# ZhengyiLuo/UHC

Measured on AMD Instinct MI355X. Metric: env-steps/sec (69-DoF SMPL humanoid, 15 substeps/step), higher is better.
Workload: dtype f64

## Files before the change

### __graft_entry__.py

```python
import os
import subprocess
import sys

ROOT = os.path.dirname(os.path.abspath(__file__))
CSRC = os.path.join(ROOT, "uhc_amd", "csrc")
LIB = os.path.join(CSRC, "libuhc_amd.so")
HIP_SOURCES = ["uhc_k_fast.hip", "uhc_k_fast_dense.hip", "uhc_k_fast_fwd.hip", "uhc_k_fast_fwd_dense.hip", "uhc_k_general.hip", "uhc_k_general_fwd.hip", "uhc_k_big.hip", "uhc_k_big_fwd.hip", "uhc_k_general_q.hip", "uhc_k_big_q.hip", "uhc_k_huge_q.hip",
               "uhc_batch_kernels.hip", "uhc_env.hip", "uhc_rollout.hip", "uhc_plan.cpp", "uhc_capi.cpp", "uhc_env_capi.cpp"]
HIP_HEADERS = ["uhc_physics_impl.h", "uhc_primal.h", "uhc_mpr.h", "uhc_device.h", "uhc_device_env.h", "uhc_host.h", "uhc_plan.h", "uhc_launch.h"]


def _stale(out, deps):
    return (not os.path.exists(out)) or any(os.path.getmtime(d) > os.path.getmtime(out) for d in deps)


def compile_lib(lib=LIB, extra_flags=(), force=False, obj_dir=None):
    from concurrent.futures import ThreadPoolExecutor
    hipcc = os.environ.get("HIPCC", "/opt/rocm/bin/hipcc")
    obj_dir = obj_dir or os.path.join(CSRC, "build")
    os.makedirs(obj_dir, exist_ok=True)
    abi = os.path.join(ROOT, "include", "uhc_amd.h")

    def deps(src):
        if src.startswith("uhc_k_"):
            big = ["uhc_primal.h"] if src.startswith(("uhc_k_big", "uhc_k_huge")) else []
            return [os.path.join(CSRC, h) for h in ["uhc_physics_impl.h", "uhc_mpr.h", "uhc_device.h", "uhc_launch.h"] + big] + [abi]
        if src == "uhc_batch_kernels.hip":
            return [os.path.join(CSRC, h) for h in ["uhc_physics_impl.h", "uhc_mpr.h", "uhc_device.h"]] + [abi]
        if src in ("uhc_env.hip", "uhc_env_capi.cpp"):
            return [os.path.join(CSRC, "uhc_device_env.h"), abi]
        if src in ("uhc_plan.cpp", "uhc_capi.cpp"):
            return [os.path.join(CSRC, h) for h in ["uhc_plan.h", "uhc_host.h", "uhc_device.h"] + (["uhc_launch.h"] if src == "uhc_capi.cpp" else [])] + [abi]
        return [abi]

    flags = ["--offload-arch=gfx950", "-O3", "-std=c++17", "-fPIC", "-fvisibility=hidden", "-Wno-unused-value"] + list(extra_flags)
    import hashlib

    def key_of(src):
        h = hashlib.sha256(" ".join(flags).encode())
        for f in [os.path.join(CSRC, src)] + deps(src):
            h.update(open(f, "rb").read())
        return h.hexdigest()

    jobs = []
    for src in HIP_SOURCES:
        sp, ob = os.path.join(CSRC, src), os.path.join(obj_dir, src + ".o")
        key = key_of(src)
        have = open(ob + ".key").read() if os.path.exists(ob + ".key") and os.path.exists(ob) else None
        if force or have != key:
            jobs.append(([hipcc] + flags + ["-c", sp, "-o", ob], ob, key))

    def run(job):
        cmd, ob, key = job
        if os.path.exists(ob + ".key"):
            os.remove(ob + ".key")
        rc = subprocess.call(cmd, cwd=CSRC)
        if rc == 0:
            open(ob + ".key", "w").write(key)
        return rc

    if jobs:
        with ThreadPoolExecutor(max_workers=min(len(jobs), os.cpu_count() or 1)) as ex:
            for rc, job in zip(ex.map(run, jobs), jobs):
                if rc != 0:
                    raise RuntimeError("hipcc failed: " + " ".join(job[0]))
    objs = [os.path.join(obj_dir, src + ".o") for src in HIP_SOURCES]
    if force or jobs or _stale(lib, objs):
        subprocess.check_call([hipcc, "--offload-arch=gfx950", "-shared", "-fPIC", "-fvisibility=hidden", "-o", lib] + objs, cwd=CSRC)


def build(force: bool = False) -> None:
    if ROOT not in sys.path:
        sys.path.insert(0, ROOT)
    compile_lib(force=force)
    from oracle.build import build as build_oracle
    build_oracle(force=force)
    import uhc_amd
    from uhc_amd import _lib
    L = _lib.lib()
    for s in _lib.SYMBOLS:
        getattr(L, s)
    lint()


def lint() -> None:
    out = os.path.join(CSRC, "build", "isa_lint.txt")
    if os.path.exists(out) and os.path.getmtime(out) >= os.path.getmtime(LIB):
        txt = open(out).read()
    else:
        r = subprocess.run([sys.executable, os.path.join(ROOT, "tools", "isa_lint.py"), LIB], capture_output=True, text=True)
# ... 52 lines not shown
```

### uhc_amd/csrc/uhc_capi.cpp

```cpp
#include <hip/hip_runtime.h>

#include <algorithm>
#include <cstdarg>
#include <cstdio>
#include <cstdlib>
#include <cstring>
#include <memory>
#include <string>
#include <vector>

#include "uhc_host.h"
#include "uhc_launch.h"
#include "uhc_plan.h"

static const UhcStepInstance g_steps[] = UHC_STEP_TABLE;
static hipError_t uhc_launch_step(int mode, int tier, const KernelArgs* A, const double* d_action, const double* d_tbase, const int* d_active,
                                  size_t lds_bytes, hipStream_t stream) {
    const bool queue = A->list != nullptr;
    if (queue) { mode = 0; tier = tier == 4 ? 4 : tier == 3 ? 3 : 2; }
    else if (tier == 3) mode = mode == 0 ? 0 : 1;
    else if (tier != 1) { tier = 2; mode = mode == 0 ? 0 : mode == 1 ? 1 : 2; }
    else mode = mode == 2 ? 2 : mode == 0 ? 0 : 1;
    const bool dense = tier != 1 || (mode != 2 && (A->cf.ndense > 0 || A->ball_limits));
    for (const UhcStepInstance& s : g_steps)
        if (s.queue == queue && s.tier == tier && s.mode == mode && s.dense == dense) return s.launch(A, d_action, d_tbase, d_active, lds_bytes, stream);
    return hipErrorInvalidDeviceFunction;
}
static hipError_t uhc_set_lds_limit(size_t lds_bytes, size_t lds_bytes_fast, size_t lds_bytes_big) {
    const size_t bytes[3] = {lds_bytes, lds_bytes_fast, lds_bytes_big};
    for (const UhcStepInstance& s : g_steps) {
        if (s.lds == 2 && !lds_bytes_big) continue;
        const hipError_t e = s.set_lds(bytes[s.lds]);
        if (e != hipSuccess) return e;
    }
    return hipSuccess;
}
extern "C" hipError_t uhc_launch_tier_lists(const int* tier, const int* d_active, int n_env, int* tier_now, int* lists, int* counts, int* cursors, int* fin,
                                            const int* cost, const int* fresh, int* order, int launch4, int* pend3, hipStream_t stream);
extern "C" hipError_t uhc_launch_gate(const int* started, int want, int* waited, long long* trace, hipStream_t stream);
extern "C" hipError_t uhc_launch_set_state(const DevState* s, int nq, int nv, int nu, const int* env_ids, int n,
                                           const double* qpos, const double* qvel, int* mask, hipStream_t stream);

static thread_local std::string g_err;
static int fail(const char* fmt, ...) {
    char buf[1024];
    va_list ap;
    va_start(ap, fmt);
    vsnprintf(buf, sizeof buf, fmt, ap);
    va_end(ap);
    g_err = buf;
    return 1;
}
#define HIP_OK(expr)                                                                      \
    do {                                                                                  \
        hipError_t e__ = (expr);                                                          \
        if (e__ != hipSuccess) return fail("%s: %s", #expr, hipGetErrorString(e__));      \
    } while (0)

extern "C" const char* uhc_last_error(void) { return g_err.c_str(); }
extern "C" int32_t uhc_abi_version(void) { return UHC_ABI_VERSION; }
extern "C" int32_t uhc_build_flags(void) {
    int32_t f = 0;
#ifdef UHC_EXPERIMENTS
    f |= 1;
#endif
#ifdef UHC_STAGE_PROF
    f |= 2;
#endif
#ifdef UHC_POISON_LDS
    f |= 4;
#endif
#ifdef UHC_GUARD_LDS
    f |= 8;
#endif
    return f;
}

template <class T>
static void take(std::vector<T>& v, const T*& p, size_t n) {
    v.assign(p, p + n);
    if (v.empty()) v.push_back(T());
    p = v.data();
}

extern "C" int32_t uhc_model_create(const UhcModelDesc* in, UhcModel** out) {
    if (!in || !out) return fail("uhc_model_create: null argument");
    if (in->nbody < 1 || in->nbody > UHC_WAVE) return fail("uhc_model_create: nbody=%d outside [1,64]", in->nbody);
    if (in->nv < 1 || in->nv > 2 * UHC_WAVE) return fail("uhc_model_create: nv=%d outside [1,128]", in->nv);
    if (in->njnt > 2 * UHC_WAVE) return fail("uhc_model_create: njnt=%d > 128", in->njnt);
    UhcModel* m = new UhcModel();
    m->d = *in;
    UhcModelDesc& d = m->d;
    const size_t nb = d.nbody, nj = d.njnt, nv = d.nv, ng = d.ngeom;
    take(m->body_parentid, d.body_parentid, nb); take(m->body_jntadr, d.body_jntadr, nb);
    take(m->body_jntnum, d.body_jntnum, nb); take(m->body_dofadr, d.body_dofadr, nb); take(m->body_dofnum, d.body_dofnum, nb);
    take(m->body_pos, d.body_pos, 3 * nb); take(m->body_quat, d.body_quat, 4 * nb); take(m->body_ipos, d.body_ipos, 3 * nb);
    take(m->body_iquat, d.body_iquat, 4 * nb); take(m->body_mass, d.body_mass, nb); take(m->body_inertia, d.body_inertia, 3 * nb);
    take(m->body_invweight0, d.body_invweight0, 2 * nb);
    take(m->jnt_type, d.jnt_type, nj); take(m->jnt_bodyid, d.jnt_bodyid, nj); take(m->jnt_qposadr, d.jnt_qposadr, nj);
    take(m->jnt_dofadr, d.jnt_dofadr, nj); take(m->jnt_limited, d.jnt_limited, nj);
    take(m->jnt_pos, d.jnt_pos, 3 * nj); take(m->jnt_axis, d.jnt_axis, 3 * nj); take(m->jnt_range, d.jnt_range, 2 * nj);
    take(m->jnt_stiffness, d.jnt_stiffness, nj); take(m->jnt_margin, d.jnt_margin, nj);
    take(m->qpos0, d.qpos0, d.nq); take(m->qpos_spring, d.qpos_spring, d.nq);
    take(m->dof_bodyid, d.dof_bodyid, nv); take(m->dof_jntid, d.dof_jntid, nv); take(m->dof_parentid, d.dof_parentid, nv);
    take(m->dof_madr, d.dof_madr, nv + 1);
    take(m->dof_armature, d.dof_armature, nv); take(m->dof_damping, d.dof_damping, nv);
    take(m->dof_frictionloss, d.dof_frictionloss, nv); take(m->dof_invweight0, d.dof_invweight0, nv);
    take(m->geom_type, d.geom_type, ng); take(m->geom_bodyid, d.geom_bodyid, ng); take(m->geom_contype, d.geom_contype, ng);
    take(m->geom_conaffinity, d.geom_conaffinity, ng); take(m->geom_condim, d.geom_condim, ng);
    take(m->geom_vertadr, d.geom_vertadr, ng); take(m->geom_vertnum, d.geom_vertnum, ng);
    take(m->geom_pos, d.geom_pos, 3 * ng); take(m->geom_quat, d.geom_quat, 4 * ng); take(m->geom_size, d.geom_size, 3 * ng);
    take(m->geom_friction, d.geom_friction, 3 * ng); take(m->geom_margin, d.geom_margin, ng); take(m->geom_gap, d.geom_gap, ng);
    take(m->geom_solref, d.geom_solref, 2 * ng); take(m->geom_solimp, d.geom_solimp, 5 * ng);
    take(m->geom_rbound, d.geom_rbound, ng); take(m->geom_center, d.geom_center, 3 * ng);
    take(m->mesh_vert, d.mesh_vert, 3 * (size_t)d.nmeshvert);
    take(m->mesh_adjadr, d.mesh_adjadr, (size_t)d.nmeshvert + 1); take(m->mesh_adj, d.mesh_adj, d.nmeshadj);
    take(m->exclude_pair, d.exclude_pair, 2 * (size_t)d.nexclude);
    take(m->actuator_dofid, d.actuator_dofid, d.nu); take(m->actuator_gear, d.actuator_gear, 3 * (size_t)d.nu);
    for (size_t b = 1; b < nb; b++)
        if (d.body_parentid[b] >= (int)b) { delete m; return fail("uhc_model_create: bodies must be in depth-first order"); }
    for (size_t i = 0; i < nv; i++)
        if (d.dof_parentid[i] >= (int)i) { delete m; return fail("uhc_model_create: dofs must be in depth-first order"); }
    *out = m;
    return 0;
}
extern "C" void uhc_model_free(UhcModel* m) { delete m; }
extern "C" int32_t uhc_model_nM(const UhcModel* m) { return m ? m->d.dof_madr[m->d.nv] : -1; }

template <class T>
static int upload(UhcBatch* b, const std::vector<T>& h, const T** dptr) {
    void* p = nullptr;
    size_t bytes = std::max<size_t>(h.size(), 1) * sizeof(T);
    HIP_OK(hipMalloc(&p, bytes));
    b->allocs.push_back(p);
    if (!h.empty()) HIP_OK(hipMemcpy(p, h.data(), h.size() * sizeof(T), hipMemcpyHostToDevice));
    *dptr = (const T*)p;
    return 0;
}
template <class T>
static int dalloc(UhcBatch* b, size_t n, T** dptr) {
    void* p = nullptr;
    const size_t bytes = std::max<size_t>(n, 1) * sizeof(T);
    if (b->hbm_guard) {
        HIP_OK(hipMalloc(&p, bytes + 512));
        HIP_OK(hipMemset(p, 0xA5, bytes + 512));
        HIP_OK(hipMemset((char*)p + 256, 0, bytes));
        b->allocs.push_back(p);
        b->fences.push_back({(char*)p, bytes});
        *dptr = (T*)((char*)p + 256);
        return 0;
    }
    HIP_OK(hipMalloc(&p, bytes));
    HIP_OK(hipMemset(p, 0, bytes));
    b->allocs.push_back(p);
    *dptr = (T*)p;
    return 0;
}
#define TRY(x) do { if (x) return 1; } while (0)


static int upload_plan(UhcBatch* b, const BatchPlan& P, const UhcModelDesc& d, const UhcCtrlDesc* ctrl, const int32_t* h_env_model) {
    KernelArgs& A = b->A;
    DevTopo& T = A.t;
    const int nb = d.nbody, nv = d.nv, nj = d.njnt, ng = d.ngeom;
    auto ivec = [](const int32_t* p, size_t n) { return std::vector<int>(p, p + n); };
    TRY(upload(b, ivec(d.body_parentid, nb), &T.body_parentid)); TRY(upload(b, ivec(d.body_jntadr, nb), &T.body_jntadr));
    TRY(upload(b, ivec(d.body_jntnum, nb), &T.body_jntnum)); TRY(upload(b, ivec(d.body_dofadr, nb), &T.body_dofadr));
    TRY(upload(b, ivec(d.body_dofnum, nb), &T.body_dofnum)); TRY(upload(b, P.body_rootid, &T.body_rootid));
    TRY(upload(b, P.body_nsub, &T.body_nsub)); TRY(upload(b, P.body_lastdof, &T.body_lastdof)); TRY(upload(b, P.body_depth, &T.body_depth));
    TRY(upload(b, ivec(d.jnt_type, nj), &T.jnt_type)); TRY(upload(b, ivec(d.jnt_bodyid, nj), &T.jnt_bodyid));
    TRY(upload(b, ivec(d.jnt_qposadr, nj), &T.jnt_qposadr)); TRY(upload(b, ivec(d.jnt_dofadr, nj), &T.jnt_dofadr));
    TRY(upload(b, ivec(d.jnt_limited, nj), &T.jnt_limited));
    TRY(upload(b, ivec(d.dof_bodyid, nv), &T.dof_bodyid)); TRY(upload(b, ivec(d.dof_jntid, nv), &T.dof_jntid));
    TRY(upload(b, ivec(d.dof_parentid, nv), &T.dof_parentid)); TRY(upload(b, ivec(d.dof_madr, nv + 1), &T.dof_madr));
    TRY(upload(b, P.dof_depth, &T.dof_depth)); TRY(upload(b, P.dof_ndesc, &T.dof_ndesc));
    TRY(upload(b, P.dof_anc, &T.dof_anc)); TRY(upload(b, P.ncommon, &T.dof_ncommon)); TRY(upload(b, P.m_row, &T.m_row)); TRY(upload(b, P.m_col, &T.m_col)); TRY(upload(b, P.m_ij, &T.m_ij));
    TRY(upload(b, ivec(d.geom_type, ng), &T.geom_type)); TRY(upload(b, ivec(d.geom_bodyid, ng), &T.geom_bodyid));
    TRY(upload(b, ivec(d.geom_condim, ng), &T.geom_condim)); TRY(upload(b, ivec(d.geom_vertadr, ng), &T.geom_vertadr));
    TRY(upload(b, ivec(d.geom_vertnum, ng), &T.geom_vertnum));
    TRY(upload(b, P.pg1, &T.pair_g1)); TRY(upload(b, P.pg2, &T.pair_g2));
    TRY(upload(b, P.cg1, &T.cpair_g1)); TRY(upload(b, P.cg2, &T.cpair_g2)); TRY(upload(b, P.dof_rootid, &T.dof_rootid));
    TRY(upload(b, ivec(d.actuator_dofid, d.nu), &T.actuator_dofid));
    TRY(upload(b, P.model_blob, &A.s.model_blob));
    if (h_env_model) TRY(upload(b, std::vector<int>(h_env_model, h_env_model + b->n_env), &A.s.env_model));
    else if (b->n_models > 1) TRY(upload(b, std::vector<int>(b->n_env, 0), &A.s.env_model));
    if (A.c.rfc_mode == 2) TRY(upload(b, P.vf_body, &A.c.vf_body));
    auto dvec = [&](const double* p) { return std::vector<double>(p, p + d.nu); };
    TRY(upload(b, dvec(ctrl->jkp), &A.c.jkp)); TRY(upload(b, dvec(ctrl->jkd), &A.c.jkd));
    TRY(upload(b, dvec(ctrl->torque_lim), &A.c.torque_lim)); TRY(upload(b, dvec(ctrl->a_scale), &A.c.a_scale));
    if (!P.guard_tab.empty()) {
        const std::vector<int>& tab = P.guard_tab;
        int* d_tab = nullptr;
        TRY(dalloc(b, tab.size(), &d_tab)); TRY(dalloc(b, 4, &b->d_guard_hits));
        HIP_OK(hipMemcpy(d_tab, tab.data(), tab.size() * sizeof(int), hipMemcpyHostToDevice));
        HIP_OK(hipMemset(b->d_guard_hits, 0, 4 * sizeof(int)));
        A.guard_tab = d_tab; A.guard_hits = b->d_guard_hits;
        fprintf(stderr, "uhc guard: LDS guard words on -- fast %d + %d, general %d + %d, large %d + %d, tier 4 %d + %d (persistent + constraint phase)\n", tab[0], tab[1],
                tab[64], tab[65], tab[128], tab[129], tab[192], tab[193]);
    }
    TRY(upload(b, P.chain, &T.chain));
    TRY(upload(b, P.dof_act, &T.dof_act));
    TRY(upload(b, P.fac_prog, &T.fac_prog)); TRY(upload(b, P.sol_back, &T.sol_back)); TRY(upload(b, P.sol_fwd, &T.sol_fwd));
    return 0;
}

static int alloc_state(UhcBatch* b, const UhcModel* const* models, const int32_t* h_env_model) {
    KernelArgs& A = b->A;
    DevState& S = A.s;
    const size_t E = b->n_env;
    const int nq = A.t.nq, nv = A.t.nv, nu = A.t.nu, nb = A.t.nbody;
    TRY(dalloc(b, E * nq, &S.qpos)); TRY(dalloc(b, E * nv, &S.qvel)); TRY(dalloc(b, E * nv, &S.qacc)); TRY(dalloc(b, E * nv, &S.qacc_ws));
    TRY(dalloc(b, E * 3 * nb, &S.xpos)); TRY(dalloc(b, E * 4 * nb, &S.xquat)); TRY(dalloc(b, E * 3 * nb, &S.xipos));
    TRY(dalloc(b, 4, &S.path_stats));
    TRY(dalloc(b, E * A.t.nM, &S.qM)); TRY(dalloc(b, 6 * E + 1, &S.redo)); S.pend2 = S.redo + E; S.pend3 = S.redo + 2 * E; S.resume = S.redo + 3 * E; S.why = S.redo + 4 * E; TRY(dalloc(b, 2, &S.q_abort));
    A.chunk_done = S.redo + 5 * E; A.ticket = S.redo + 6 * E; TRY(dalloc(b, E * UHC_CHUNK_REC, &A.chunk_rec));
    TRY(dalloc(b, E, &S.tier)); TRY(dalloc(b, E, &b->tier_now)); S.tier_now = b->tier_now; TRY(dalloc(b, E, &S.cost));
    if (!(A.dbg & 8)) TRY(dalloc(b, E, &b->d_order));
    TRY(dalloc(b, 3 * E, &b->d_lists)); TRY(dalloc(b, 8, &b->d_counts)); TRY(dalloc(b, 8, &b->d_cursors)); TRY(dalloc(b, 8, &b->d_fin));
    { std::vector<int> one(E, 1); HIP_OK(hipMemcpy(S.tier, one.data(), E * sizeof(int), hipMemcpyHostToDevice)); } TRY(dalloc(b, E, &S.fresh)); TRY(dalloc(b, E * 40, &S.prof)); TRY(dalloc(b, E * nv, &S.bias)); TRY(dalloc(b, E * nu, &S.ctrl));
    TRY(dalloc(b, E * nv, &S.applied));
    if (A.c.rfc_mode == 2) { TRY(dalloc(b, E * 6 * nv, &S.cdof)); TRY(dalloc(b, E * 3 * nb, &S.rootcom)); }
    TRY(dalloc(b, E, &S.ncon)); TRY(dalloc(b, E, &S.nefc)); TRY(dalloc(b, E, &S.fail)); TRY(dalloc(b, E, &S.solver_iter));
    TRY(dalloc(b, E, &S.overflow));
    if (A.last_tier == 4) { TRY(dalloc(b, E * (size_t)A.gy_stride, &A.gY)); TRY(dalloc(b, E * (size_t)A.gd_stride, &A.gD)); }
    TRY(dalloc(b, E, &b->reset_mask));
    {
        std::vector<double> q0(E * nq);
        for (size_t e = 0; e < E; e++) {
            const UhcModelDesc& md = models[h_env_model ? h_env_model[e] : 0]->d;
            memcpy(&q0[e * nq], md.qpos0, nq * sizeof(double));
        }
        HIP_OK(hipMemcpy(S.qpos, q0.data(), q0.size() * sizeof(double), hipMemcpyHostToDevice));
    }
    const int64_t n = (int64_t)E;
    const UhcBatch::Field fields[21] = {{S.qpos, n * nq}, {S.qvel, n * nv}, {S.xpos, n * 3 * nb}, {S.xquat, n * 4 * nb}, {S.xipos, n * 3 * nb}, {S.qM, n * A.t.nM}, {S.bias, n * nv},
                                        {S.qacc, n * nv}, {S.ctrl, n * nu}, {S.ncon, n}, {S.nefc, n}, {S.fail, n}, {S.solver_iter, n}, {S.applied, n * nv}, {S.overflow, n},
                                        {S.prof, n * 40}, {S.redo, n}, {S.tier, n}, {S.why, n}, {S.qacc_ws, n * nv}, {S.cost, n}};
    std::copy(fields, fields + 21, b->field);
    return 0;
}

extern "C" void uhc_batch_free(UhcBatch* b);
extern "C" int32_t uhc_batch_create(const UhcModel* const* models, int32_t n_models, const int32_t* h_env_model, int32_t n_env,
                                    int32_t device_id, const UhcCtrlDesc* ctrl, UhcBatch** out) {
    if (!out) return fail("uhc_batch_create: bad argument");
    const BatchKnobs knobs = read_knobs();
    BatchPlan P;
    std::string err;
    if (plan_batch(models, n_models, h_env_model, n_env, ctrl, knobs, &P, &err)) return fail("%s", err.c_str());
    int ndev = 0;
    HIP_OK(hipGetDeviceCount(&ndev));
    if (device_id < 0 || device_id >= ndev) return fail("uhc_batch_create: device %d not present (%d devices)", device_id, ndev);
    HIP_OK(hipSetDevice(device_id));

    std::unique_ptr<UhcBatch, void (*)(UhcBatch*)> owner(new UhcBatch(), uhc_batch_free);
    UhcBatch* b = owner.get();
    b->n_env = n_env;
    b->device = device_id;
    b->n_models = n_models;
    b->n_trailing_free = P.n_trailing_free;
    b->A = P.A;
    b->nM = P.A.t.nM;
    b->lds_bytes = P.lds_bytes; b->lds_bytes_fast = P.lds_bytes_fast; b->lds_bytes_big = P.lds_bytes_big;
    b->use_fast = P.use_fast;
    b->hbm_guard = knobs.guard != 0;
    b->q2_div = knobs.q2_div; b->q2_wait_min = knobs.q2_wait_min; b->q2_max = knobs.q2_max; b->q3_max = knobs.q3_max; b->q4_max = knobs.q4_max;
    b->fast_chunk = (P.A.dbg & 4) ? 0x7fff : knobs.fast_chunk;
    TRY(upload_plan(b, P, models[0]->d, ctrl, h_env_model));
    HIP_OK(uhc_set_lds_limit(b->lds_bytes, b->lds_bytes_fast, b->lds_bytes_big));
    TRY(alloc_state(b, models, h_env_model));
    HIP_OK(hipStreamCreateWithFlags(&b->own_stream, hipStreamNonBlocking));
    b->stream = b->own_stream;
    *out = owner.release();
    return 0;
}

static void guard_report(UhcBatch* b) {
    if (!b->d_guard_hits) return;
    int h[4] = {0, 0, 0, 0};
    if (hipMemcpy(h, b->d_guard_hits, sizeof(h), hipMemcpyDeviceToHost) != hipSuccess) return;
    if (h[0] > b->guard_reported) {
        b->guard_reported = h[0];
        fprintf(stderr, "uhc guard: %d LDS guard words OVERWRITTEN so far; the first: tier %d, %s region %d (offset %d doubles), env %d\n", h[0], h[1] >> 16,
                ((h[1] >> 8) & 0xff) ? "constraint-phase" : "persistent", h[1] & 0xff, h[3], h[2]);
    }
}
extern "C" void uhc_batch_free(UhcBatch* b) {
    if (!b) return;
    hipSetDevice(b->device);
    hipDeviceSynchronize();
    guard_report(b);
    if (!b->fences.empty()) {
        int bad = 0;
        unsigned char h[512];
        for (size_t k = 0; k < b->fences.size(); k++) {
            const auto& f = b->fences[k];
            bool hit = false;
            if (hipMemcpy(h, f.first, 256, hipMemcpyDeviceToHost) != hipSuccess || hipMemcpy(h + 256, f.first + 256 + f.second, 256, hipMemcpyDeviceToHost) != hipSuccess) continue;
            for (int i = 0; i < 512; i++) hit = hit || h[i] != 0xA5;
            if (hit) { if (!bad) fprintf(stderr, "uhc guard: HBM array %zu (%zu bytes) has an OVERWRITTEN fence\n", k, f.second); bad++; }
        }
        fprintf(stderr, "uhc guard: %zu fenced HBM arrays checked, %d with an overwritten fence\n", b->fences.size(), bad);
    }
    if (b->d_guard_hits) fprintf(stderr, "uhc guard: batch of %d envs freed, %d guard words overwritten in its lifetime\n", b->n_env, b->guard_reported);
    for (void* p : b->allocs) hipFree(p);
    for (auto& ev : b->ev_used) { hipEventDestroy(ev.first); hipEventDestroy(ev.second); }
    for (auto& ev : b->ev_free) { hipEventDestroy(ev.first); hipEventDestroy(ev.second); }
    for (hipEvent_t e : {b->ev_fork, b->ev_side1, b->ev_side2, b->ev_side3}) if (e) hipEventDestroy(e);
    for (hipEvent_t e : b->cnt_ev) if (e) hipEventDestroy(e);
    if (b->h_counts) hipHostFree(b->h_counts);
    if (b->side_stream) hipStreamDestroy(b->side_stream);
    if (b->side_stream3) hipStreamDestroy(b->side_stream3);
    if (b->side_stream4) hipStreamDestroy(b->side_stream4);
    if (b->own_stream) hipStreamDestroy(b->own_stream);
    delete b;
}
extern "C" int32_t uhc_batch_set_stream(UhcBatch* b, void* s) {
    if (!b) return fail("uhc_batch_set_stream: null batch");
    b->stream = (hipStream_t)s;
    return 0;
}
extern "C" int32_t uhc_batch_sync(UhcBatch* b) {
    if (!b) return fail("uhc_batch_sync: null batch");
    HIP_OK(hipStreamSynchronize(b->stream));
    guard_report(b);
    return 0;
}
extern "C" int32_t uhc_batch_set_rfc_scale(UhcBatch* b, double s) {
    if (!b) return fail("uhc_batch_set_rfc_scale: null batch");
    b->A.c.rfc_scale = s;
    return 0;
}
extern "C" int32_t uhc_batch_set_kernel_path(UhcBatch* b, int32_t mode) {
    if (!b) return fail("uhc_batch_set_kernel_path: null batch");
    if (mode < 0 || mode > 2) return fail("uhc_batch_set_kernel_path: mode %d (0 fast then general, 1 general only, 2 adaptive)", mode);
    b->general_only = mode == 1;
    b->path_mode = mode;
    if (mode == 2 && !b->side_stream) {
        HIP_OK(hipSetDevice(b->device));
        int least = 0, greatest = 0;
        HIP_OK(hipDeviceGetStreamPriorityRange(&least, &greatest));
        HIP_OK(hipStreamCreateWithPriority(&b->side_stream, hipStreamNonBlocking, greatest));
        HIP_OK(hipStreamCreateWithPriority(&b->side_stream3, hipStreamNonBlocking, (least != greatest && least != 0) ? least : greatest));
        b->large_first = least != greatest && least != 0;
        { hipDeviceProp_t pr; HIP_OK(hipGetDeviceProperties(&pr, b->device)); b->n_cu = pr.multiProcessorCount > 0 ? pr.multiProcessorCount : 256; }
        HIP_OK(hipHostMalloc((void**)&b->h_counts, sizeof(int) * 8 * 8, hipHostMallocDefault));
        memset(b->h_counts, 0, sizeof(int) * 8 * 8);
        for (int k = 0; k < 8; k++) HIP_OK(hipEventCreateWithFlags(&b->cnt_ev[k], hipEventDisableTiming));
        HIP_OK(hipEventCreateWithFlags(&b->ev_fork, hipEventDisableTiming));
        HIP_OK(hipEventCreateWithFlags(&b->ev_side1, hipEventDisableTiming));
        HIP_OK(hipEventCreateWithFlags(&b->ev_side2, hipEventDisableTiming));
        HIP_OK(hipStreamCreateWithPriority(&b->side_stream4, hipStreamNonBlocking, (least != greatest && least != 0) ? least : greatest));
        HIP_OK(hipEventCreateWithFlags(&b->ev_side3, hipEventDisableTiming));
    }
    return 0;
}
extern "C" int32_t uhc_batch_set_solver(UhcBatch* b, int32_t solver, int32_t iterations) {
    if (!b || (solver != 0 && solver != 1)) return fail("uhc_batch_set_solver: solver must be 0 (sweeps) or 1 (active set)");
    b->A.t.solver = solver;
    if (iterations > 0) b->A.t.iterations = iterations;
    return 0;
}
extern "C" int32_t uhc_batch_field(UhcBatch* b, int32_t f, void** p, int64_t* n) {
    if (!b || f < 0 || f > 20 || !b->field[f].ptr) return fail("uhc_batch_field: unknown field %d", f);
    if (p) *p = b->field[f].ptr;
    if (n) *n = b->field[f].count;
    return 0;
}
static int launch_sticky(UhcBatch* b, int mode, const double* d_action, const double* d_tbase, const int* d_active, bool timed, std::pair<hipEvent_t, hipEvent_t> ev) {
    const bool big = b->A.last_tier >= 3;
        KernelArgs K = b->A;
        int est4 = 0, est2_then = 0;
        if (b->A.last_tier == 4 && b->q4_max > 0)
            for (long long k = b->cnt_step - 1; k >= 0 && k > b->cnt_step - 8; k--)
                if (hipEventQuery(b->cnt_ev[k % 8]) == hipSuccess) { est4 = b->h_counts[8 * (k % 8) + 7]; est2_then = b->h_counts[8 * (k % 8) + 2]; break; }
        (void)hipGetLastError();
    StickyInputs in{};
    in.est4 = est4; in.est2_then = est2_then; in.n_env = b->n_env; in.n_cu = b->n_cu; in.lds_bytes_fast = b->lds_bytes_fast; in.large_first = b->large_first;
    in.fast_chunk = b->fast_chunk; in.n_substeps = b->A.c.n_substeps;
    in.last_tier = b->A.last_tier; in.q2_div = b->q2_div; in.q2_wait_min = b->q2_wait_min; in.q2_max = b->q2_max; in.q3_max = b->q3_max; in.q4_max = b->q4_max;
#ifdef UHC_EXPERIMENTS
    in.fixed_cap2 = (b->A.dbg & 2048) != 0;
#endif
    in.queues_off = b->queues_off;
    const bool launch4 = plan_sticky_step(in).launch4;
        K.cnt4 = b->d_counts + 7;
        HIP_OK(uhc_launch_tier_lists(b->A.s.tier, d_active, b->n_env, b->tier_now, b->d_lists, b->d_counts, b->d_cursors, b->d_fin, b->A.s.cost, b->A.s.fresh, b->d_order,
                                     launch4 ? 1 : 0, b->A.s.pend3, b->stream));
        HIP_OK(hipEventRecord(b->ev_fork, b->stream));
        if (b->cnt_step >= 2) HIP_OK(hipEventSynchronize(b->cnt_ev[(b->cnt_step - 2) % 8]));
        int est2 = 0, est3 = 0, handed2 = 0;
        for (long long k = b->cnt_step - 1; k >= 0 && k > b->cnt_step - 8; k--)
            if (hipEventQuery(b->cnt_ev[k % 8]) == hipSuccess) {
                const int* hc = b->h_counts + 8 * (k % 8);
                est2 = hc[2]; est3 = hc[3]; handed2 = std::max(0, hc[2] - hc[4]);
                if (b->A.dbg & 64) fprintf(stderr, "uhc step %lld: queues %d / %d envs (%d handed on), gate waited %.1f us, gave up %d, queues_off %d\n", k, est2, est3, handed2, 0.01 * hc[1], hc[0], (int)b->queues_off);
                if (hc[0] > b->aborts_seen) {
                    b->aborts_seen = hc[0];
                    b->queues_off_until = ++b->abort_events >= 3 ? (long long)1 << 62 : b->cnt_step + 32;
                }
                b->queues_off = b->cnt_step < b->queues_off_until;
                break;
            }
    in.est2 = est2; in.est3 = est3; in.handed2 = handed2; in.queues_off = b->queues_off;
    const StickySizes z = plan_sticky_step(in);
    const bool queues = z.queues, waiting = z.waiting, q3 = z.q3, q4 = launch4 && q3;
    const int grid2 = z.grid2, grid3 = z.grid3, grid4 = z.grid4;
    K.sticky_mask = (queues ? 4 : 0) | (q3 ? 8 : 0) | (launch4 ? 16 : 0);
        if (q4) {
            HIP_OK(hipStreamWaitEvent(b->side_stream4, b->ev_fork, 0));
            K.tier_want = 0; K.list = b->d_lists + 2 * b->n_env; K.list_count = b->d_counts + 6; K.list_cursor = b->d_cursors + 4;
            K.grid = grid4; K.n_wait = grid4; K.spares = nullptr; K.started = nullptr;
            K.prod_fin = b->d_fin + 5; K.prod_total = grid3;
            K.fin = nullptr; K.q_next = nullptr; K.q_next_count = nullptr;
            if (b->A.dbg & 64) fprintf(stderr, "uhc step %lld: %d tier-4 consumers (%d env-steps went through tier 4 when last seen)\n", b->cnt_step, grid4, est4);
            HIP_OK(uhc_launch_step(mode, 4, &K, d_action, d_tbase, nullptr, b->lds_bytes_big, b->side_stream4));
            HIP_OK(hipEventRecord(b->ev_side3, b->side_stream4));
        }
        auto launch_large = [&]() -> int {
            HIP_OK(hipStreamWaitEvent(b->side_stream3, b->ev_fork, 0));
            K.tier_want = 0; K.list = b->d_lists + b->n_env; K.list_count = b->d_counts + 3; K.list_cursor = b->d_cursors + 3;
            K.grid = grid3; K.n_wait = grid3; K.spares = nullptr; K.started = b->d_fin + 4;
            K.prod_fin = b->d_fin + 2; K.prod_total = grid2;
            K.fin = q4 ? b->d_fin + 5 : nullptr; K.q_next = q4 ? b->d_lists + 2 * b->n_env : nullptr; K.q_next_count = q4 ? b->d_counts + 6 : nullptr;
            HIP_OK(uhc_launch_step(mode, 3, &K, d_action, d_tbase, nullptr, b->lds_bytes_big, b->side_stream3));
            HIP_OK(hipEventRecord(b->ev_side2, b->side_stream3));
            return 0;
        };
        if (q3 && b->large_first) { if (launch_large()) return -1; }
        if (queues) {
            HIP_OK(hipStreamWaitEvent(b->side_stream, b->ev_fork, 0));
            if (q3 && b->large_first && !(b->A.dbg & 32)) HIP_OK(uhc_launch_gate(b->d_fin + 4, grid3, nullptr, nullptr, b->side_stream));
            K.tier_want = 0; K.list = b->d_lists; K.list_count = b->d_counts + 2; K.list_cursor = b->d_cursors + 2;
            K.grid = grid2;
            K.prod_fin = waiting ? b->d_fin + 1 : nullptr; K.prod_total = z.fast.prod_total;
            K.fin = b->d_fin + 2; K.started = waiting ? b->d_fin + 3 : nullptr;
            K.n_wait = z.n_wait; K.spares = b->d_fin;
            K.q_next = q3 ? b->d_lists + b->n_env : nullptr; K.q_next_count = q3 ? b->d_counts + 3 : nullptr;
            HIP_OK(uhc_launch_step(mode, 2, &K, d_action, d_tbase, nullptr, b->lds_bytes, b->side_stream));
            HIP_OK(hipEventRecord(b->ev_side1, b->side_stream));
        }
        if (q3 && !b->large_first) { if (launch_large()) return -1; }
        K.list = nullptr; K.list_count = nullptr; K.list_cursor = nullptr; K.grid = 0; K.prod_fin = nullptr; K.prod_total = 0; K.started = nullptr; K.spares = nullptr;
        if (waiting && !(b->A.dbg & 32)) HIP_OK(uhc_launch_gate(b->d_fin + 3, grid2, b->d_counts + 1,
                                                                     (b->A.dbg & 16) ? b->A.s.prof + (size_t)(b->n_env - 1) * 40 + 16 : nullptr, b->stream));
        K.tier_want = 1;
        K.chunk = z.fast.chunk; K.grid = z.fast.chunk ? z.fast.grid : 0;
        K.order = b->d_order;
        K.fin = waiting ? b->d_fin + 1 : nullptr;
        K.q_next = waiting ? b->d_lists : nullptr; K.q_next_count = waiting ? b->d_counts + 2 : nullptr;
        if (timed) HIP_OK(hipEventRecord(ev.first, b->stream));
        HIP_OK(uhc_launch_step(mode, 1, &K, d_action, d_tbase, d_active, b->lds_bytes_fast, b->stream));
        if (timed) { HIP_OK(hipEventRecord(ev.second, b->stream)); b->ev_used.push_back(ev); }
        K.tier_want = 0; K.sticky_mask = 0; K.fin = nullptr; K.q_next = nullptr; K.q_next_count = nullptr; K.order = nullptr; K.chunk = 0; K.grid = 0;
        if (queues) HIP_OK(hipStreamWaitEvent(b->stream, b->ev_side1, 0));
        HIP_OK(uhc_launch_step(mode, 2, &K, d_action, d_tbase, b->A.s.pend2, b->lds_bytes, b->stream));
        if (q3) HIP_OK(hipStreamWaitEvent(b->stream, b->ev_side2, 0));
        if (q4) HIP_OK(hipStreamWaitEvent(b->stream, b->ev_side3, 0));
        if (big) HIP_OK(uhc_launch_step(mode, 3, &K, d_action, d_tbase, b->A.s.pend3, b->lds_bytes_big, b->stream));
        const int slot = (int)(b->cnt_step % 8);
        HIP_OK(hipMemcpyAsync(b->d_counts, b->A.s.q_abort, sizeof(int), hipMemcpyDeviceToDevice, b->stream));
        HIP_OK(hipMemcpyAsync(b->h_counts + 8 * slot, b->d_counts, 8 * sizeof(int), hipMemcpyDeviceToHost, b->stream));
        HIP_OK(hipEventRecord(b->cnt_ev[slot], b->stream));
        b->cnt_step++;
        return 0;
    }

static int launch(UhcBatch* b, int mode, const double* d_action, const double* d_tbase, const int* d_active) {
    std::pair<hipEvent_t, hipEvent_t> ev{nullptr, nullptr};
    const bool timed = b->timing && mode == 0;
    if (timed) {
        if (b->ev_free.empty()) { HIP_OK(hipEventCreate(&ev.first)); HIP_OK(hipEventCreate(&ev.second)); }
        else { ev = b->ev_free.back(); b->ev_free.pop_back(); }
    }
    const bool general = b->general_only;
    const bool big = b->A.last_tier >= 3;
    HIP_OK(hipMemsetAsync(b->A.s.redo, 0, sizeof(int) * ((size_t)b->n_env * 6 + 1), b->stream));
    bool capturing = false;
    {
        hipStreamCaptureStatus cs = hipStreamCaptureStatusNone;
        if (hipStreamIsCapturing(b->stream, &cs) == hipSuccess) capturing = cs == hipStreamCaptureStatusActive;
        else (void)hipGetLastError();
    }
    if (mode == 0 && b->path_mode == 2 && b->use_fast && !general && !capturing) return launch_sticky(b, mode, d_action, d_tbase, d_active, timed, ev);
    if (b->use_fast && !general) {
        if (timed) HIP_OK(hipEventRecord(ev.first, b->stream));
        KernelArgs K = b->A;
        if (mode == 0) {
            const FastChunks f = plan_fast_chunks(K.c.n_substeps, default_fast_chunk(b->fast_chunk, K.c.n_substeps, b->n_env, b->n_cu, b->lds_bytes_fast), b->n_env);
            K.chunk = f.chunk; K.grid = f.chunk ? f.grid : 0;
        }
        HIP_OK(uhc_launch_step(mode, 1, &K, d_action, d_tbase, d_active, b->lds_bytes_fast, b->stream));
        if (timed) { HIP_OK(hipEventRecord(ev.second, b->stream)); b->ev_used.push_back(ev); }
        HIP_OK(uhc_launch_step(mode, 2, &b->A, d_action, d_tbase, b->A.s.pend2, b->lds_bytes, b->stream));
    } else {
        if (timed) HIP_OK(hipEventRecord(ev.first, b->stream));
        HIP_OK(uhc_launch_step(mode, 2, &b->A, d_action, d_tbase, d_active, b->lds_bytes, b->stream));
        if (timed) { HIP_OK(hipEventRecord(ev.second, b->stream)); b->ev_used.push_back(ev); }
    }
    if (big) HIP_OK(uhc_launch_step(mode, 3, &b->A, d_action, d_tbase, b->A.s.pend3, b->lds_bytes_big, b->stream));
    return 0;
}

extern "C" int32_t uhc_batch_set_overflow_mode(UhcBatch* b, int32_t truncate) {
    if (!b) return fail("uhc_batch_set_overflow_mode: null batch");
    b->A.truncate = truncate != 0;
    return 0;
}
extern "C" int32_t uhc_batch_set_timing(UhcBatch* b, int32_t enable) {
    if (!b) return fail("uhc_batch_set_timing: null batch");
    b->timing = enable != 0;
    return 0;
}
extern "C" int32_t uhc_batch_kernel_time(UhcBatch* b, double* total_ms, int32_t* launches) {
    if (!b || !total_ms || !launches) return fail("uhc_batch_kernel_time: null argument");
    double tot = 0;
    for (auto& ev : b->ev_used) {
        float ms = 0;
        HIP_OK(hipEventSynchronize(ev.second));
        HIP_OK(hipEventElapsedTime(&ms, ev.first, ev.second));
        tot += ms;
        b->ev_free.push_back(ev);
// ... 62 lines not shown
```

### uhc_amd/csrc/uhc_device.h

```cpp
#pragma once
#include <hip/hip_runtime.h>
#include <stdint.h>

#define UHC_WAVE 64
#define UHC_FAST_MAXEFC 64
#define UHC_FAST_MAXCON 16
#define UHC_FAST_MAXCON_DENSE 24
#define UHC_FAST_MAXTWO 12
#define UHC_GEN_MAXEFC 128
#define UHC_GEN_MAXCON 64
#define UHC_GEN_MAXTWO 20
#define UHC_BIG_MAXEFC 256
#define UHC_BIG_MAXCON 128
#define UHC_BIG_MAXTWO 32
#define UHC_MAXTWO 32
#define UHC_HUGE_MAXEFC 1024
#define UHC_HUGE_MAXCON 192
#define UHC_HUGE_MAXCON_MOST 320
#define UHC_HUGE_MAXTWO 128
#define UHC_DOF_MAXACT 4
#define UHC_CON_STRIDE 24
#define UHC_WHY_CONTACTS (1 << 16)
#define UHC_WHY_ROWS (1 << 17)
#define UHC_WHY_DENSE_SLOTS (1 << 18)
// ... 76 lines not shown
    int* q_abort;
    int* tier;
    const int* tier_now;
    int* cost;
    int* fresh;
    const int* env_model;
    long long* prof;
    unsigned long long* path_stats;
    const double* model_blob;
};

#define UHC_PRIMAL_WAVES 4
#define UHC_PRIMAL_CLS_STRIDE 144
struct PrimalScratch { int anc, stY, dstage, pair_all, pair_cls, pair_cnt, cw, mbx, part, runs, total; };
__host__ __device__ inline PrimalScratch primal_scratch(int nv, int YS) {
    PrimalScratch p;
    int o = 0;
    auto take = [&](int n) { const int at = o; o += (n + 1) & ~1; return at; };
    p.anc = take((nv * YS + 3) / 4 + 1);
    p.stY = take(UHC_PRIMAL_WAVES * 16 * 32);
    p.dstage = take(nv * 8);
    p.pair_all = take(528 / 4);
    p.pair_cls = take(4 * UHC_PRIMAL_CLS_STRIDE / 4);
    p.pair_cnt = take((4 * 33 + 3) / 4);
    p.cw = take(UHC_PRIMAL_WAVES * 32);
    p.mbx = take(4);
    p.part = take(UHC_PRIMAL_WAVES * 128);
    p.runs = take(UHC_HUGE_MAXEFC / 2);
    p.total = o;
    return p;
}

struct TierCap {
    int maxefc, maxcon;
    int ndense;
    int ycap;
    int vstage;
    int ld_delta;
};
struct KernelArgs {
    DevTopo t;
    DevNumOff o;
    DevLds lf;
    DevLds l;
    DevLds lh;
    DevLds lx;
    TierCap cf, cg, ch, cx;
    double* gY;
    double* gD;
    int gy_stride, gd_stride;
    int last_tier;
    const int* order;
    int tier_want;
    int sticky_mask;
    int* list;
    int* list_count;
    int* list_cursor;
    const int* prod_fin;
    int prod_total;
    int n_wait;
    int* spares;
    int* started;
    int* fin;
    int* q_next;
    int* q_next_count;
    const int* guard_tab;
    int* guard_hits;
    int* cnt4;
    int grid;
    int marks[8];
    int t4_rows;
    int truncate;
    int ball_limits;
    int dbg;
    int nvp;
    int adjdeg;
    DevCtrl c;
    DevState s;
    int n_env;
    int chunk;
    int* ticket;
    int* chunk_done;
    int* chunk_rec;
};
#define UHC_CHUNK_ALL 0x7fff
#define UHC_CHUNK_ABANDON (1 << 30)
#define UHC_CHUNK_TAKEN (1 << 29)
#define UHC_CHUNK_CLOSING (1 << 28)
#define UHC_CHUNK_REC 16
```

### uhc_amd/csrc/uhc_host.h

```cpp
#pragma once
#include <hip/hip_runtime.h>

#include <cstdint>
#include <utility>
#include <vector>

#include "../../include/uhc_amd.h"
#include "uhc_device.h"

struct UhcModel {
    UhcModelDesc d;
    std::vector<int32_t> body_parentid, body_jntadr, body_jntnum, body_dofadr, body_dofnum;
    std::vector<double> body_pos, body_quat, body_ipos, body_iquat, body_mass, body_inertia, body_invweight0;
    std::vector<int32_t> jnt_type, jnt_bodyid, jnt_qposadr, jnt_dofadr, jnt_limited;
    std::vector<double> jnt_pos, jnt_axis, jnt_range, jnt_stiffness, jnt_margin, qpos0, qpos_spring;
    std::vector<int32_t> dof_bodyid, dof_jntid, dof_parentid, dof_madr;
    std::vector<double> dof_armature, dof_damping, dof_frictionloss, dof_invweight0;
    std::vector<int32_t> geom_type, geom_bodyid, geom_contype, geom_conaffinity, geom_condim, geom_vertadr, geom_vertnum;
    std::vector<double> geom_pos, geom_quat, geom_size, geom_friction, geom_margin, geom_gap, geom_solref, geom_solimp,
        geom_rbound, geom_center, mesh_vert;
    std::vector<int32_t> mesh_adjadr, mesh_adj, exclude_pair, actuator_dofid;
    std::vector<double> actuator_gear;
};

struct UhcBatch {
    int n_env = 0, device = 0;
    hipStream_t own_stream = nullptr, stream = nullptr;
    KernelArgs A;
    size_t lds_bytes = 0, lds_bytes_fast = 0, lds_bytes_big = 0;
    bool use_fast = true;
    bool general_only = false;
    int path_mode = 0;
    hipStream_t side_stream = nullptr, side_stream3 = nullptr, side_stream4 = nullptr;
    hipEvent_t ev_fork = nullptr, ev_side1 = nullptr, ev_side2 = nullptr, ev_side3 = nullptr;
    int* tier_now = nullptr;
    bool large_first = false;
    int n_cu = 256;
    std::vector<std::pair<char*, size_t>> fences;
    int* d_guard_hits = nullptr;
    int guard_reported = 0;
    int* d_order = nullptr;
    int aborts_seen = 0, abort_events = 0;
    long long queues_off_until = 0;
    int q2_wait_min = 16;
    int q2_div = 1;
    int q2_max = 256;
    int q4_max = 16;
    int q3_max = 32;
    int fast_chunk = 0;
    int *d_lists = nullptr, *d_counts = nullptr, *d_cursors = nullptr, *d_fin = nullptr;
    bool queues_off = false;
    int* h_counts = nullptr;
    hipEvent_t cnt_ev[8] = {};
    long long cnt_step = 0;
    std::vector<void*> allocs;
    int nM = 0;
    int* reset_mask = nullptr;
    bool timing = false;
    std::vector<std::pair<hipEvent_t, hipEvent_t>> ev_used, ev_free;
    int n_models = 1;
    int n_trailing_free = 0;
    bool hbm_guard = false;
    struct Field { void* ptr; int64_t count; };
    Field field[21] = {};
};
```

### uhc_amd/csrc/uhc_launch.h

```cpp
#pragma once
#include <hip/hip_runtime.h>

#include "uhc_device.h"

typedef hipError_t (*UhcStepLaunch)(const KernelArgs* A, const double* d_action, const double* d_tbase, const int* d_active, size_t lds_bytes, hipStream_t stream);
typedef hipError_t (*UhcSetLds)(size_t lds_bytes);

#define UHC_STEP_INSTANCES(X)                                                                                                                     \
    X(m0_fast, 0, 1, false, false) X(m0_fast_dense, 0, 1, true, false) X(m1_fast, 1, 1, false, false) X(m1_fast_dense, 1, 1, true, false)         \
    X(m2_fast, 2, 1, false, false) X(m0_gen, 0, 2, true, false) X(m1_gen, 1, 2, true, false) X(m2_gen, 2, 2, true, false)                         \
    X(m0_big, 0, 3, true, false) X(m1_big, 1, 3, true, false) X(m0_gen_q, 0, 2, true, true) X(m0_big_q, 0, 3, true, true) X(m0_huge_q, 0, 4, true, true)

#define UHC_DECL_LAUNCH(name, mode, tier, dense, queue)                                                                                         \
    extern "C" hipError_t uhc_launch_##name(const KernelArgs* A, const double* d_action, const double* d_tbase, const int* d_active, size_t lds_bytes, \
                                            hipStream_t stream);                                                                                 \
    extern "C" hipError_t uhc_launch_##name##_lds(size_t lds_bytes);
UHC_STEP_INSTANCES(UHC_DECL_LAUNCH)

#define UHC_DEFINE_LAUNCH(name, KERNEL, MODE, TIER, DENSE, THREADS, GRID, ...)                                                                        \
    extern "C" hipError_t uhc_launch_##name(const KernelArgs* A, const double* d_action, const double* d_tbase, const int* d_active, size_t lds_bytes, \
                                            hipStream_t stream) {                                                                                     \
        (void)d_active;                                                                                                                               \
        hipLaunchKernelGGL((KERNEL<MODE, TIER, DENSE>), dim3(GRID), dim3(THREADS), lds_bytes, stream, *A, d_action, d_tbase, ##__VA_ARGS__);          \
        return hipGetLastError();                                                                                                                     \
    }                                                                                                                                                 \
    extern "C" hipError_t uhc_launch_##name##_lds(size_t lds_bytes) {                                                                                 \
        return hipFuncSetAttribute((const void*)KERNEL<MODE, TIER, DENSE>, hipFuncAttributeMaxDynamicSharedMemorySize, (int)lds_bytes);               \
    }
#define UHC_ENV_LAUNCH(name, MODE, TIER, DENSE) UHC_DEFINE_LAUNCH(name, uhc_step_kernel, MODE, TIER, DENSE, UHC_WAVE, A->grid ? A->grid : A->n_env, d_active)
#define UHC_QUEUE_LAUNCH(name, TIER, THREADS) UHC_DEFINE_LAUNCH(name, uhc_step_queue_kernel, 0, TIER, true, THREADS, A->grid)

struct UhcStepInstance { int mode, tier; bool dense, queue; UhcStepLaunch launch; UhcSetLds set_lds; int lds; };
#define UHC_INSTANCE_ROW(name, mode, tier, dense, queue) {mode, tier, dense, queue, uhc_launch_##name, uhc_launch_##name##_lds, tier == 1 ? 1 : tier == 2 ? 0 : 2},
#define UHC_STEP_TABLE {UHC_STEP_INSTANCES(UHC_INSTANCE_ROW)}
```

### uhc_amd/csrc/uhc_mpr.h

```cpp
#pragma once

#define UHC_CCD_EPS 2.220446049250313e-16
#define UHC_MPR_TOLERANCE 1e-6
#define UHC_MPR_MAXIT 50
#define UHC_MPR_MAXSUP 256

struct V3 { double x, y, z; };
__device__ __forceinline__ V3 v3(double x, double y, double z) { V3 r = {x, y, z}; return r; }
__device__ __forceinline__ V3 operator-(const V3& a, const V3& b) { return v3(a.x - b.x, a.y - b.y, a.z - b.z); }
__device__ __forceinline__ V3 operator+(const V3& a, const V3& b) { return v3(a.x + b.x, a.y + b.y, a.z + b.z); }
__device__ __forceinline__ V3 operator*(const V3& a, double s) { return v3(a.x * s, a.y * s, a.z * s); }
__device__ __forceinline__ V3 neg(const V3& a) { return v3(-a.x, -a.y, -a.z); }
__device__ __forceinline__ double vdot(const V3& a, const V3& b) { return a.x * b.x + a.y * b.y + a.z * b.z; }
__device__ __forceinline__ V3 vcross(const V3& a, const V3& b) { return v3(a.y * b.z - a.z * b.y, a.z * b.x - a.x * b.z, a.x * b.y - a.y * b.x); }
__device__ __forceinline__ V3 vnorm(const V3& a) { const double n = sqrt(vdot(a, a)); return v3(a.x / n, a.y / n, a.z / n); }
__device__ __forceinline__ V3 vsel(bool c, const V3& a, const V3& b) { return v3(c ? a.x : b.x, c ? a.y : b.y, c ? a.z : b.z); }
__device__ __forceinline__ bool ccd_zero(double x) { return fabs(x) < UHC_CCD_EPS; }
__device__ __forceinline__ bool ccd_eq(double a, double b) {
    const double ab = fabs(a - b);
    if (ab < UHC_CCD_EPS) return true;
    a = fabs(a); b = fabs(b);
    return b > a ? ab < UHC_CCD_EPS * b : ab < UHC_CCD_EPS * a;
}

// ... 312 lines not shown
                    pair_support_wave2(VB, Ap, Aq, a, b, a2, b2v);
                    const bool mq = LANE == q;
                    v4.v = vsel(mq, a2 - b2v, v4.v);
                    v4.s = vsel(mq, a2 + b2v, v4.s);
                    const bool mine = LANE == p;
                    v4.v = vsel(mine, a - b, v4.v);
                    v4.s = vsel(mine, a + b, v4.s);
                    continue;
                }
            }
            pair_support_wave(VB, Ap.R1, Ap.P1, Ap.voff1, Ap.vn1, Ap.R2, Ap.P2, Ap.voff2, Ap.vn2, Ap.d, Ap.hm1, Ap.hm2, a, b);
            const bool mine = LANE == p;
            v4.v = vsel(mine, a - b, v4.v);
            v4.s = vsel(mine, a + b, v4.s);
        }
        bool to_refine = false, to_pen = false;
        if (st == MPR_D1) {
            p1 = v4;
            dt = vdot(p1.v, dir);
            if (ccd_zero(dt) || dt < 0) st = MPR_DONE;
            else {
                dir = vcross(p0.v, p1.v);
                if (ccd_zero(vdot(dir, dir))) {
                    if (ccd_eq(p1.v.x, 0) && ccd_eq(p1.v.y, 0) && ccd_eq(p1.v.z, 0)) { M.depth = 0; M.dir = v3(0, 0, 0); }
                    else { M.depth = sqrt(vdot(p1.v, p1.v)); M.dir = vnorm(p1.v); }
                    M.pos = v3(0.5 * p1.s.x, 0.5 * p1.s.y, 0.5 * p1.s.z);
                    M.hit = true;
                    st = MPR_DONE;
                } else { dir = vnorm(dir); st = MPR_D2; }
            }
        } else if (st == MPR_D2) {
            p2 = v4;
            dt = vdot(p2.v, dir);
            if (ccd_zero(dt) || dt < 0) st = MPR_DONE;
            else {
                dir = vnorm(vcross(p1.v - p0.v, p2.v - p0.v));
                if (vdot(dir, p0.v) > 0) { const CcdSup t = p1; p1 = p2; p2 = t; dir = neg(dir); }
                st = MPR_D3;
            }
        } else if (st == MPR_D3) {
            dt = vdot(v4.v, dir);
            if (ccd_zero(dt) || dt < 0) st = MPR_DONE;
            else {
                bool cont = false;
                dt = vdot(vcross(p1.v, v4.v), p0.v);
                if (dt < 0 && !ccd_zero(dt)) { p2 = v4; cont = true; }
                if (!cont) {
                    dt = vdot(vcross(v4.v, p2.v), p0.v);
                    if (dt < 0 && !ccd_zero(dt)) { p1 = v4; cont = true; }
                }
                if (cont) dir = vnorm(vcross(p1.v - p0.v, p2.v - p0.v));
                else { p3 = v4; to_refine = true; }
            }
        } else if (st == MPR_REFINE) {
            dt = vdot(v4.v, dir);
            if (!(ccd_zero(dt) || dt > 0) || portal_reach_tolerance(p1, p2, p3, v4, dir)) st = MPR_DONE;
            else { expand_portal(p0, p1, p2, p3, v4); to_refine = true; }
        } else if (st == MPR_PEN) {
            if (portal_reach_tolerance(p1, p2, p3, v4, dir) || it > UHC_MPR_MAXIT) {
                V3 pd;
                M.depth = sqrt(point_tri_dist2(p1.v, p2.v, p3.v, pd));
                if (ccd_zero(pd.x) && ccd_zero(pd.y) && ccd_zero(pd.z)) pd = dir;
                M.dir = vnorm(pd);
                M.pos = find_pos(p0, p1, p2, p3);
                M.hit = true;
                st = MPR_DONE;
            } else {
                expand_portal(p0, p1, p2, p3, v4);
                it++;
                dir = portal_dir(p1, p2, p3);
            }
        }
        if (to_refine) {
            dir = portal_dir(p1, p2, p3);
            dt = vdot(dir, p1.v);
            if (ccd_zero(dt) || dt > 0) to_pen = true;
            else st = MPR_REFINE;
        }
        if (to_pen) { dir = portal_dir(p1, p2, p3); it = 0; st = MPR_PEN; }
    }
}

#if defined(UHC_NW2)
enum { MCMD_EXIT = 0, MCMD_ROUND = 1, MCMD_ROWS = 2 };
struct MprMB { int* hdr; double* io[6]; double* hm1; double* hm2; int* st4; int* st2; };
template <int TIER>
__device__ __forceinline__ MprMB mpr_mb(const KernelArgs& A, double* S) {
    const DevLds& L = lds_of<TIER>(A);
    MprMB m;
    m.hdr = (int*)(S + L.rowR);
    m.io[0] = S + L.rowR + 4;
    m.io[1] = S + L.rowAref; m.io[2] = S + L.rowAref + UHC_WAVE;
    m.io[3] = S + L.rowB; m.io[4] = S + L.rowB + UHC_WAVE;
    m.io[5] = S + L.rowF; m.hm1 = S + L.rowF + UHC_WAVE;
    m.st4 = (int*)(S + L.rowDa); m.st2 = (int*)(S + L.rowW); m.hm2 = S + L.rowW + UHC_WAVE;
    return m;
}
__device__ __forceinline__ SupArgs mpr_mb_args(const MprMB& MB, const double* xmat, const double* xpos, int p) {
    SupArgs a;
    const int b1 = __builtin_amdgcn_readfirstlane(MB.st4[4 * p]), b2 = __builtin_amdgcn_readfirstlane(MB.st4[4 * p + 1]);
    a.R1 = xmat + 9 * b1; a.P1 = xpos + 3 * b1; a.R2 = xmat + 9 * b2; a.P2 = xpos + 3 * b2;
    a.voff1 = __builtin_amdgcn_readfirstlane(MB.st4[4 * p + 2]); a.vn1 = __builtin_amdgcn_readfirstlane(MB.st4[4 * p + 3]);
    a.voff2 = __builtin_amdgcn_readfirstlane(MB.st2[2 * p]); a.vn2 = __builtin_amdgcn_readfirstlane(MB.st2[2 * p + 1]);
    a.hm1 = MB.hm1[p]; a.hm2 = MB.hm2[p];
    a.d = v3(MB.io[0][p], MB.io[1][p], MB.io[2][p]);
    return a;
}
__device__ __forceinline__ void mpr_mb_put(const MprMB& MB, int p, const V3& a, const V3& b) {
    if (LANE == 0) {
        MB.io[0][p] = a.x - b.x; MB.io[1][p] = a.y - b.y; MB.io[2][p] = a.z - b.z; MB.io[3][p] = a.x + b.x; MB.io[4][p] = a.y + b.y; MB.io[5][p] = a.z + b.z;
    }
}
__device__ __forceinline__ void mpr_serve_round(const double* __restrict__ VB, const double* __restrict__ xmat, const double* __restrict__ xpos, const MprMB& MB, unsigned long long live, int wid, int nw) {
    const int n = __builtin_popcountll(live), h = (n + nw - 1) / nw;
    int take = min(h, n - wid * h);
    for (int k = 0; k < wid * h && live; k++) live &= live - 1;
    while (live && take > 0) {
        const int p = __ffsll((long long)live) - 1;
        live &= live - 1;
        const SupArgs Ap = mpr_mb_args(MB, xmat, xpos, p);
        V3 a, b;
        if (take >= 2 && live && UHC_MPR_PAIRWISE) {
            const int q = __ffsll((long long)live) - 1;
            const SupArgs Aq = mpr_mb_args(MB, xmat, xpos, q);
            if (max(max(Ap.vn1, Ap.vn2), max(Aq.vn1, Aq.vn2)) <= UHC_WAVE) {
                live &= live - 1;
                take -= 2;
                V3 a2, b2v;
                pair_support_wave2(VB, Ap, Aq, a, b, a2, b2v);
                mpr_mb_put(MB, p, a, b);
                mpr_mb_put(MB, q, a2, b2v);
                continue;
            }
        }
        pair_support_wave(VB, Ap.R1, Ap.P1, Ap.voff1, Ap.vn1, Ap.R2, Ap.P2, Ap.voff2, Ap.vn2, Ap.d, Ap.hm1, Ap.hm2, a, b);
        mpr_mb_put(MB, p, a, b);
        take -= 1;
    }
}
template <bool LDSV>
__device__ __forceinline__ void mpr_wave_mw(const double* __restrict__ VB, const double* __restrict__ xmat, const double* __restrict__ xpos, bool active, MprLane& M, const MprMB& MB, int vstage,
                                            const double* vb_global) {
    CcdSup p0, p1, p2, p3, v4;
    V3 dir = v3(0, 0, 0);
    double dt;
    int st = MPR_DONE, it = 0;
    M.hit = false; M.depth = 0; M.dir = v3(0, 0, 0); M.pos = v3(0, 0, 0);
    p0.v = p0.s = p1.v = p1.s = p2.v = p2.s = p3.v = p3.s = v4.v = v4.s = v3(0, 0, 0);
    if (active) {
        p0.s = M.c1 + M.c2; p0.v = M.c1 - M.c2;
        if (ccd_eq(p0.v.x, 0) && ccd_eq(p0.v.y, 0) && ccd_eq(p0.v.z, 0)) p0.v.x += UHC_CCD_EPS * 10;
        dir = vnorm(neg(p0.v));
        st = MPR_D1;
        MB.st4[4 * LANE] = M.b1; MB.st4[4 * LANE + 1] = M.b2; MB.st4[4 * LANE + 2] = M.voff1; MB.st4[4 * LANE + 3] = M.vn1;
        MB.st2[2 * LANE] = M.voff2; MB.st2[2 * LANE + 1] = M.vn2;
        MB.hm1[LANE] = M.hm1; MB.hm2[LANE] = M.hm2;
    }
    int* mbi = MB.hdr;
    if (LANE == 0) {
        mbi[3] = LDSV ? vstage : -1;
        mbi[4] = (int)((unsigned long long)vb_global & 0xffffffffull); mbi[5] = (int)((unsigned long long)vb_global >> 32);
    }
    for (int round = 0;; round++) {
        const unsigned long long live = __builtin_amdgcn_ballot_w64(st != MPR_DONE);
        if (!live || round == UHC_MPR_MAXSUP) break;
        if (st != MPR_DONE) { MB.io[0][LANE] = dir.x; MB.io[1][LANE] = dir.y; MB.io[2][LANE] = dir.z; }
        if (LANE == 0) { mbi[0] = MCMD_ROUND; mbi[1] = (int)(live & 0xffffffffull); mbi[2] = (int)(live >> 32); }
        __syncthreads();
        mpr_serve_round(VB, xmat, xpos, MB, live, 0, UHC_NWG);
        __syncthreads();
        if (st != MPR_DONE) { v4.v = v3(MB.io[0][LANE], MB.io[1][LANE], MB.io[2][LANE]); v4.s = v3(MB.io[3][LANE], MB.io[4][LANE], MB.io[5][LANE]); }
        bool to_refine = false, to_pen = false;
        if (st == MPR_D1) {
            p1 = v4;
            dt = vdot(p1.v, dir);
            if (ccd_zero(dt) || dt < 0) st = MPR_DONE;
            else {
                dir = vcross(p0.v, p1.v);
                if (ccd_zero(vdot(dir, dir))) {
                    if (ccd_eq(p1.v.x, 0) && ccd_eq(p1.v.y, 0) && ccd_eq(p1.v.z, 0)) { M.depth = 0; M.dir = v3(0, 0, 0); }
                    else { M.depth = sqrt(vdot(p1.v, p1.v)); M.dir = vnorm(p1.v); }
                    M.pos = v3(0.5 * p1.s.x, 0.5 * p1.s.y, 0.5 * p1.s.z);
                    M.hit = true;
                    st = MPR_DONE;
                } else { dir = vnorm(dir); st = MPR_D2; }
            }
        } else if (st == MPR_D2) {
            p2 = v4;
            dt = vdot(p2.v, dir);
            if (ccd_zero(dt) || dt < 0) st = MPR_DONE;
            else {
                dir = vnorm(vcross(p1.v - p0.v, p2.v - p0.v));
                if (vdot(dir, p0.v) > 0) { const CcdSup t = p1; p1 = p2; p2 = t; dir = neg(dir); }
                st = MPR_D3;
            }
        } else if (st == MPR_D3) {
            dt = vdot(v4.v, dir);
            if (ccd_zero(dt) || dt < 0) st = MPR_DONE;
            else {
                bool cont = false;
                dt = vdot(vcross(p1.v, v4.v), p0.v);
                if (dt < 0 && !ccd_zero(dt)) { p2 = v4; cont = true; }
                if (!cont) {
                    dt = vdot(vcross(v4.v, p2.v), p0.v);
                    if (dt < 0 && !ccd_zero(dt)) { p1 = v4; cont = true; }
                }
                if (cont) dir = vnorm(vcross(p1.v - p0.v, p2.v - p0.v));
                else { p3 = v4; to_refine = true; }
            }
        } else if (st == MPR_REFINE) {
            dt = vdot(v4.v, dir);
            if (!(ccd_zero(dt) || dt > 0) || portal_reach_tolerance(p1, p2, p3, v4, dir)) st = MPR_DONE;
            else { expand_portal(p0, p1, p2, p3, v4); to_refine = true; }
        } else if (st == MPR_PEN) {
            if (portal_reach_tolerance(p1, p2, p3, v4, dir) || it > UHC_MPR_MAXIT) {
                V3 pd;
                M.depth = sqrt(point_tri_dist2(p1.v, p2.v, p3.v, pd));
                if (ccd_zero(pd.x) && ccd_zero(pd.y) && ccd_zero(pd.z)) pd = dir;
                M.dir = vnorm(pd);
                M.pos = find_pos(p0, p1, p2, p3);
                M.hit = true;
                st = MPR_DONE;
            } else {
                expand_portal(p0, p1, p2, p3, v4);
                it++;
                dir = portal_dir(p1, p2, p3);
            }
        }
        if (to_refine) {
            dir = portal_dir(p1, p2, p3);
            dt = vdot(dir, p1.v);
            if (ccd_zero(dt) || dt > 0) to_pen = true;
            else st = MPR_REFINE;
        }
        if (to_pen) { dir = portal_dir(p1, p2, p3); it = 0; st = MPR_PEN; }
    }
}
template <int TIER>
__device__ __forceinline__ void mpr_helper(const KernelArgs& A, double* S) {
    const DevLds& L = lds_of<TIER>(A);
    const MprMB MB = mpr_mb<TIER>(A, S);
    const int* mbi = MB.hdr;
    const int wid = __builtin_amdgcn_readfirstlane((int)(threadIdx.x >> 6));
    const LaneConst HLC = lane_const<true>(A.t);
    for (;;) {
        __syncthreads();
        const int cmd = __builtin_amdgcn_readfirstlane(mbi[0]);
        if (cmd == MCMD_EXIT) return;
        if (cmd == MCMD_ROWS) {
            const int nefc = __builtin_amdgcn_readfirstlane(mbi[1]), ntwo = __builtin_amdgcn_readfirstlane(mbi[2]);
            const unsigned long long mbp = ((unsigned long long)(unsigned)__builtin_amdgcn_readfirstlane(mbi[5]) << 32) | (unsigned)__builtin_amdgcn_readfirstlane(mbi[4]);
            __syncthreads();
            if (ntwo > 0) k_dense_groups<TIER>(A, S, HLC, S + L.dense, ntwo, 1, 2);
            __syncthreads();
            if (UHC_WAVE + LANE < nefc) k_row_one<TIER>(A, (const double*)mbp, S, UHC_WAVE + LANE, S + L.Y);
            __syncthreads();
            continue;
        }
        const unsigned long long live = ((unsigned long long)(unsigned)__builtin_amdgcn_readfirstlane(mbi[2]) << 32) | (unsigned)__builtin_amdgcn_readfirstlane(mbi[1]);
        const int vst = __builtin_amdgcn_readfirstlane(mbi[3]);
        if (vst >= 0) mpr_serve_round(S + vst, S + L.xmat, S + L.xpos, MB, live, wid, UHC_NWG);
        else {
            const unsigned long long vb = ((unsigned long long)(unsigned)__builtin_amdgcn_readfirstlane(mbi[5]) << 32) | (unsigned)__builtin_amdgcn_readfirstlane(mbi[4]);
            mpr_serve_round((const double*)vb, S + L.xmat, S + L.xpos, MB, live, wid, UHC_NWG);
        }
        __syncthreads();
    }
}
template <int TIER>
__device__ __forceinline__ void mpr_release_helpers(const KernelArgs& A, double* S) {
    int* mbi = mpr_mb<TIER>(A, S).hdr;
    if (LANE == 0) mbi[0] = MCMD_EXIT;
    __syncthreads();
}
#endif
```

### uhc_amd/csrc/uhc_physics_impl.h

```cpp
#pragma once
#include <type_traits>
#include "../../include/uhc_amd.h"
#include "uhc_device.h"

extern __shared__ __attribute__((aligned(16))) double smem[];

#if defined(UHC_NW4)
#define UHC_NWG 4
#elif defined(UHC_NW2)
#define UHC_NWG 2
#else
#define UHC_NWG 1
#endif
#if UHC_NWG > 1
#define LANE ((int)(threadIdx.x & 63u))
#else
#define LANE ((int)threadIdx.x)
#endif
#define UHC_NPROF 40
#ifdef UHC_STAGE_PROF
#define PROF_DECL long long pt_[UHC_NPROF] = {}; long long pt_last_ = __builtin_readcyclecounter();
#define PROF_ARGS , long long* pt_, long long& pt_last_
#define PROF_PASS , pt_, pt_last_
#define PROF(i) { const long long now_ = __builtin_readcyclecounter(); pt_[i] += now_ - pt_last_; pt_last_ = now_; }
#else
#define PROF_DECL
#define PROF_ARGS
#define PROF_PASS
#define PROF(i)
#endif
#ifdef UHC_EXPERIMENTS
#define UHC_EXP(bit) ((A.dbg & (bit)) != 0)
#else
#define UHC_EXP(bit) false
#endif
template <int TIER> __device__ __forceinline__ const DevLds& lds_of(const KernelArgs& A) {
    if constexpr (TIER == 1) return A.lf; else if constexpr (TIER == 2) return A.l; else if constexpr (TIER == 3) return A.lh; else return A.lx;
}
template <int TIER> __device__ __forceinline__ const TierCap& cap_of(const KernelArgs& A) {
    if constexpr (TIER == 1) return A.cf; else if constexpr (TIER == 2) return A.cg; else if constexpr (TIER == 3) return A.ch; else return A.cx;
}
template <int TIER> __device__ __forceinline__ bool hands_on(const KernelArgs& A) { return TIER == 1 ? !A.truncate : TIER < A.last_tier; }
#if UHC_NWG > 1
__device__ __forceinline__ void wsync() {
    __builtin_amdgcn_fence(__ATOMIC_RELEASE, "workgroup");
    __builtin_amdgcn_wave_barrier();
    __builtin_amdgcn_fence(__ATOMIC_ACQUIRE, "workgroup");
}
#else
__device__ __forceinline__ void wsync() { __syncthreads(); }
#endif
template <int TIER> __device__ __forceinline__ double* y_store(const KernelArgs& A, double* S, int env) {
    if constexpr (TIER == 4) return A.gY + (size_t)env * A.gy_stride; else return S + lds_of<TIER>(A).Y;
}
template <int TIER> __device__ __forceinline__ double* d_store(const KernelArgs& A, double* S, int env) {
    if constexpr (TIER == 4) return A.gD + (size_t)env * A.gd_stride; else return S + lds_of<TIER>(A).dense;
}

__device__ __forceinline__ double bcast(double v, int src) {
    int lo = __builtin_amdgcn_readlane(__double2loint(v), src);
    int hi = __builtin_amdgcn_readlane(__double2hiint(v), src);
    return __hiloint2double(hi, lo);
}
template <int CTRL>
__device__ __forceinline__ double dpp_f64(double v) {
    const int lo = __builtin_amdgcn_update_dpp(0, __double2loint(v), CTRL, 0xf, 0xf, true);
    const int hi = __builtin_amdgcn_update_dpp(0, __double2hiint(v), CTRL, 0xf, 0xf, true);
    return __hiloint2double(hi, lo);
}
#define DPP_QUAD_1032 0xB1
#define DPP_QUAD_2301 0x4E
#define DPP_ROW_HALF_MIRROR 0x141
#define DPP_ROW_MIRROR 0x140
__device__ __forceinline__ double wave_sum(double v) {
    v += dpp_f64<DPP_QUAD_1032>(v);
    v += dpp_f64<DPP_QUAD_2301>(v);
    v += dpp_f64<DPP_ROW_HALF_MIRROR>(v);
    v += dpp_f64<DPP_ROW_MIRROR>(v);
    return (bcast(v, 0) + bcast(v, 16)) + (bcast(v, 32) + bcast(v, 48));
}
__device__ __forceinline__ double wave_min(double v) {
    v = fmin(v, dpp_f64<DPP_QUAD_1032>(v));
    v = fmin(v, dpp_f64<DPP_QUAD_2301>(v));
    v = fmin(v, dpp_f64<DPP_ROW_HALF_MIRROR>(v));
    v = fmin(v, dpp_f64<DPP_ROW_MIRROR>(v));
    return fmin(fmin(bcast(v, 0), bcast(v, 16)), fmin(bcast(v, 32), bcast(v, 48)));
}
__device__ __forceinline__ int wave_or(int v) { return __builtin_amdgcn_ballot_w64(v != 0) != 0; }
template <int TIER> __device__ __forceinline__ void k_row_one(const KernelArgs& A, const double* mb, double* S, const int r, double* Yb);
struct LaneConst { int d0, d1, n0, n1, m0, m1, pk0, pk1, r0, r1; bool v0, v1; };
template <int TIER> __device__ __forceinline__ void k_dense_groups(const KernelArgs& A, double* S, const LaneConst& LC, double* Db, const int ntwo, const int first, const int stride);
template <bool DENSE> __device__ __forceinline__ LaneConst lane_const(const DevTopo& T);
#include "uhc_mpr.h"

__device__ __forceinline__ void cross3(double* r, const double* a, const double* b) {
    double r0 = a[1] * b[2] - a[2] * b[1], r1 = a[2] * b[0] - a[0] * b[2], r2 = a[0] * b[1] - a[1] * b[0];
    r[0] = r0; r[1] = r1; r[2] = r2;
}
__device__ __forceinline__ double dot3(const double* a, const double* b) { return a[0] * b[0] + a[1] * b[1] + a[2] * b[2]; }
__device__ __forceinline__ void quat_mul(double* r, const double* a, const double* b) {
    double t0 = a[0] * b[0] - a[1] * b[1] - a[2] * b[2] - a[3] * b[3];
    double t1 = a[0] * b[1] + a[1] * b[0] + a[2] * b[3] - a[3] * b[2];
    double t2 = a[0] * b[2] - a[1] * b[3] + a[2] * b[0] + a[3] * b[1];
    double t3 = a[0] * b[3] + a[1] * b[2] - a[2] * b[1] + a[3] * b[0];
    r[0] = t0; r[1] = t1; r[2] = t2; r[3] = t3;
}
__device__ __forceinline__ void quat_normalize(double* q) {
    double n = sqrt(q[0] * q[0] + q[1] * q[1] + q[2] * q[2] + q[3] * q[3]);
    if (n < UHC_MINVAL) { q[0] = 1; q[1] = q[2] = q[3] = 0; return; }
    double inv = 1.0 / n;
    q[0] *= inv; q[1] *= inv; q[2] *= inv; q[3] *= inv;
}
__device__ __forceinline__ void quat_to_mat(double* m, const double* q) {
    double w = q[0], x = q[1], y = q[2], z = q[3];
    m[0] = w * w + x * x - y * y - z * z; m[1] = 2 * (x * y - w * z); m[2] = 2 * (x * z + w * y);
    m[3] = 2 * (x * y + w * z); m[4] = w * w - x * x + y * y - z * z; m[5] = 2 * (y * z - w * x);
    m[6] = 2 * (x * z - w * y); m[7] = 2 * (y * z + w * x); m[8] = w * w - x * x - y * y + z * z;
}
__device__ __forceinline__ void mat_vec(double* r, const double* m, const double* v) {
    double t0 = m[0] * v[0] + m[1] * v[1] + m[2] * v[2];
    double t1 = m[3] * v[0] + m[4] * v[1] + m[5] * v[2];
    double t2 = m[6] * v[0] + m[7] * v[1] + m[8] * v[2];
    r[0] = t0; r[1] = t1; r[2] = t2;
}
__device__ __forceinline__ void axis_angle_quat(double* q, const double* axis, double angle) {
    double s, c;
    sincos(0.5 * angle, &s, &c);
    q[0] = c; q[1] = axis[0] * s; q[2] = axis[1] * s; q[3] = axis[2] * s;
}
__device__ __forceinline__ void cross_motion(double* r, const double* v, const double* m) {
    double a[3], b[3];
    cross3(r, v, m);
    cross3(a, v, m + 3);
    cross3(b, v + 3, m);
    r[3] = a[0] + b[0]; r[4] = a[1] + b[1]; r[5] = a[2] + b[2];
}
__device__ __forceinline__ void cross_force(double* r, const double* v, const double* f) {
    double a[3], b[3];
    cross3(a, v, f);
    cross3(b, v + 3, f + 3);
    r[0] = a[0] + b[0]; r[1] = a[1] + b[1]; r[2] = a[2] + b[2];
    cross3(r + 3, v, f + 3);
}
__device__ __forceinline__ void inert_mul(double* r, const double* I, const double* v) {
    const double *w = v, *l = v + 3, *h = I + 6;
    double hxl[3], wxh[3];
    cross3(hxl, h, l);
    cross3(wxh, w, h);
    r[0] = I[0] * w[0] + I[3] * w[1] + I[4] * w[2] + hxl[0];
    r[1] = I[3] * w[0] + I[1] * w[1] + I[5] * w[2] + hxl[1];
    r[2] = I[4] * w[0] + I[5] * w[1] + I[2] * w[2] + hxl[2];
    r[3] = I[9] * l[0] + wxh[0];
    r[4] = I[9] * l[1] + wxh[1];
    r[5] = I[9] * l[2] + wxh[2];
}
__device__ __forceinline__ double dot6(const double* a, const double* b) {
    return a[0] * b[0] + a[1] * b[1] + a[2] * b[2] + a[3] * b[3] + a[4] * b[4] + a[5] * b[5];
}
__device__ __forceinline__ double clampd(double x, double lo, double hi) { return fmin(fmax(x, lo), hi); }
__device__ __forceinline__ double max0(double x) {
    double r;
    asm("v_max_f64 %0, %1, 0" : "=v"(r) : "v"(x));
    return r;
}

template <int I, int N, class F>
__device__ __forceinline__ void static_for(F&& f) {
    if constexpr (I < N) {
        f(std::integral_constant<int, I>{});
        static_for<I + 1, N>(f);
    }
}

__device__ __forceinline__ void agpr_put(int& a, int v) { asm volatile("v_accvgpr_write_b32 %0, %1" : "=a"(a) : "v"(v)); }
__device__ __forceinline__ int agpr_get(int a) { int v; asm volatile("v_accvgpr_read_b32 %0, %1" : "=v"(v) : "a"(a)); return v; }
// ... 459 lines not shown
        const int item = LANE + UHC_WAVE * pass;
        if (item < 6 * T.nbody) {
            const int bb = item / 6, k = item - 6 * bb;
            if (bb > 0) {
                const int n = T.body_nsub[bb];
                for (int c = bb + n - 1; c >= bb; c--) sub[pass] += S[L.cfrc + 6 * c + k];
            }
        }
    }
    wsync();
    for (int pass = 0; pass < 3; pass++) {
        const int item = LANE + UHC_WAVE * pass;
        if (item >= 6 && item < 6 * T.nbody) S[L.cfrc + item] = sub[pass];
    }
    wsync();
    for (int i = LANE; i < T.nv; i += UHC_WAVE) {
        double a[6], c[6];
        const int bi = T.dof_bodyid[i];
        for (int k = 0; k < 6; k++) { a[k] = S[L.cdof + 6 * i + k]; c[k] = S[L.cfrc + 6 * bi + k]; }
        S[L.bias + i] = dot6(a, c);
    }
    wsync();
}

template <int TIER>
__device__ __forceinline__ void k_smooth(const KernelArgs& A, const double* mb, double* S, const LaneConst& LC) {
    const DevTopo& T = A.t;
    const DevLds& L = lds_of<TIER>(A);
    for (int i = LANE; i < T.nv; i += UHC_WAVE) {
        double f = -mb[A.o.dof_damping + i] * S[L.qvel + i] - S[L.bias + i] + S[L.applied + i];
        const int j = T.dof_jntid[i], jt = T.jnt_type[j];
        const double k = mb[A.o.jnt_stiffness + j];
        if (k != 0 && (jt == UHC_JNT_HINGE || jt == UHC_JNT_SLIDE)) {
            const int qa = T.jnt_qposadr[j];
            f -= k * (S[L.qpos + qa] - mb[A.o.qpos_spring + qa]);
        }
        const int comp = i - T.jnt_dofadr[j];
#pragma unroll
        for (int q = 0; q < UHC_DOF_MAXACT; q++) {
            const int a = T.dof_act[i * UHC_DOF_MAXACT + q];
            if (a >= 0) f += mb[A.o.actuator_gear + 3 * a + comp] * S[L.ctrl + a];
        }
        S[L.smooth + i] = f;
    }
    wsync();
    DofVec x;
    x.a = LANE < T.nv ? S[L.smooth + LANE] : 0.0;
    x.b = LANE + UHC_WAVE < T.nv ? S[L.smooth + LANE + UHC_WAVE] : 0.0;
    k_solve<TIER>(A, S, L.LD, x, 0, LC);
    if (LANE < T.nv) S[L.smooth + LANE] = x.a;
    if (LANE + UHC_WAVE < T.nv) S[L.smooth + LANE + UHC_WAVE] = x.b;
    wsync();
}

__device__ __forceinline__ void make_frame(double* f, const double* yh = nullptr) {
    double n = sqrt(dot3(f, f));
    f[0] /= n; f[1] /= n; f[2] /= n;
    f[3] = f[4] = f[5] = 0;
    if (f[1] < 0.5 && f[1] > -0.5) f[4] = 1; else f[5] = 1;
    if (yh) {
        const double dh = dot3(f, yh);
        const double t0 = yh[0] - f[0] * dh, t1 = yh[1] - f[1] * dh, t2 = yh[2] - f[2] * dh;
        if (sqrt(t0 * t0 + t1 * t1 + t2 * t2) >= 1e-8) { f[3] = yh[0]; f[4] = yh[1]; f[5] = yh[2]; }
    }
    const double dp = dot3(f, f + 3);
    for (int k = 0; k < 3; k++) f[3 + k] -= f[k] * dp;
    n = sqrt(dot3(f + 3, f + 3));
    f[3] /= n; f[4] /= n; f[5] /= n;
    cross3(f + 6, f, f + 3);
}
__device__ __forceinline__ double impedance(const double* si, double pos, double margin) {
    double dmin = clampd(si[0], 0.0001, 0.9999), dmax = clampd(si[1], 0.0001, 0.9999), width = si[2];
    double mid = clampd(si[3], 0.0001, 0.9999), power = si[4] < 1 ? 1 : si[4];
    if (width < UHC_MINVAL) return 0.5 * (dmin + dmax);
    const double x = fabs(pos - margin) / width;
    double y;
    if (x >= 1) return dmax;
    if (x <= 0) return dmin;
    if (power == 1) y = x;
    else if (x <= mid) y = pow(x / mid, power) * mid;
    else y = 1 - pow((1 - x) / (1 - mid), power) * (1 - mid);
    return dmin + y * (dmax - dmin);
}
struct PairConst { int g1, g2, b1, b2, va, vn, dim; };
__device__ __forceinline__ int pair_dim(const DevTopo& T, int g1, int g2) {
    return max(T.geom_condim[g1], T.geom_condim[g2]) | ((T.geom_type[g2] == UHC_GEOM_CAPSULE && T.geom_vertnum[g2] == 2) ? 256 : 0);
}
__device__ __forceinline__ PairConst pair_const(const DevTopo& T) {
    PairConst c = {0, 0, 0, 0, 0, 0, 0};
    if (LANE < T.npair) {
        c.g1 = T.pair_g1[LANE]; c.g2 = T.pair_g2[LANE];
        c.b1 = T.geom_bodyid[c.g1]; c.b2 = T.geom_bodyid[c.g2];
        c.va = T.geom_vertadr[c.g2]; c.vn = T.geom_vertnum[c.g2];
        c.dim = pair_dim(T, c.g1, c.g2);
    }
    return c;
}
__device__ __forceinline__ PairConst pair_of(const DevTopo& T, const PairConst& mine, int pi) {
    PairConst c;
    if (pi < UHC_WAVE) {
        c.g1 = __builtin_amdgcn_readlane(mine.g1, pi); c.g2 = __builtin_amdgcn_readlane(mine.g2, pi);
        c.b1 = __builtin_amdgcn_readlane(mine.b1, pi); c.b2 = __builtin_amdgcn_readlane(mine.b2, pi);
        c.va = __builtin_amdgcn_readlane(mine.va, pi); c.vn = __builtin_amdgcn_readlane(mine.vn, pi);
        c.dim = __builtin_amdgcn_readlane(mine.dim, pi);
    } else {
        c.g1 = T.pair_g1[pi]; c.g2 = T.pair_g2[pi];
        c.b1 = T.geom_bodyid[c.g1]; c.b2 = T.geom_bodyid[c.g2];
        c.va = T.geom_vertadr[c.g2]; c.vn = T.geom_vertnum[c.g2];
        c.dim = pair_dim(T, c.g1, c.g2);
    }
    return c;
}
template <int TIER>
__device__ __forceinline__ void k_write_contact(const KernelArgs& A, const double* mb, double* S, int c, int g1, int g2, int b1, int b2, int dim,
                                                const double* pos, const double* n, double dist, double margin, double gap, const double* yhint = nullptr) {
    const DevTopo& T = A.t;
    double* C = S + lds_of<TIER>(A).con + c * UHC_CON_STRIDE;
    double fr[9];
    for (int k = 0; k < 3; k++) { C[k] = pos[k]; fr[k] = n[k]; }
    make_frame(fr, yhint);
    for (int k = 0; k < 9; k++) C[3 + k] = fr[k];
    const double inc = margin - gap;
    double solref[2], solimp[5];
    for (int k = 0; k < 2; k++) solref[k] = 0.5 * (mb[A.o.geom_solref + 2 * g1 + k] + mb[A.o.geom_solref + 2 * g2 + k]);
    for (int k = 0; k < 5; k++) solimp[k] = 0.5 * (mb[A.o.geom_solimp + 5 * g1 + k] + mb[A.o.geom_solimp + 5 * g2 + k]);
    const double timeconst = fmax(solref[0], 2 * T.timestep), dampratio = solref[1];
    const double dmax = clampd(solimp[1], 0.0001, 0.9999);
    C[12] = dist; C[13] = inc;
    C[14] = fmax(mb[A.o.geom_friction + 3 * g1], mb[A.o.geom_friction + 3 * g2]);
    C[15] = 1.0 / (dmax * dmax * timeconst * timeconst * dampratio * dampratio);
    C[16] = 2.0 / (dmax * timeconst);
    C[17] = impedance(solimp, dist, inc);
    C[18] = mb[A.o.body_invweight0 + 2 * b1] + mb[A.o.body_invweight0 + 2 * b2];
    C[19] = b1; C[20] = b2; C[21] = dim;
}
__device__ __forceinline__ double ball_limit(const double* qp, const double* range, double* jac) {
    double q[4] = {qp[0], qp[1], qp[2], qp[3]}, ax[3] = {1, 0, 0};
    quat_normalize(q);
    double sn = sqrt(q[1] * q[1] + q[2] * q[2] + q[3] * q[3]);
    if (sn < UHC_MINVAL) sn = 0; else { ax[0] = q[1] / sn; ax[1] = q[2] / sn; ax[2] = q[3] / sn; }
    double ang = 2 * atan2(sn, q[0]);
    if (ang > M_PI) ang -= 2 * M_PI;
    double value = fabs(ang), sg = ang < 0 ? -1.0 : 1.0;
    if (value < UHC_MINVAL) { ax[0] = 1; ax[1] = ax[2] = 0; sg = 1; value = 0; }
    for (int k = 0; k < 3; k++) jac[k] = -sg * ax[k];
    return fmax(range[0], range[1]) - value;
}
template <int TIER, bool DENSE>
__device__ __forceinline__ int k_collision(const KernelArgs& A, const double* mb, double* S, int* overflow, const PairConst& PC PROF_ARGS) {
    const DevTopo& T = A.t;
    const DevLds& L = lds_of<TIER>(A);
    int ncon = 0;
    for (int p0 = 0; p0 < T.npair; p0 += UHC_WAVE) {
        const int p = p0 + LANE;
        bool keep = false;
        if (p < T.npair) {
            PairConst P = PC;
            if (p0 > 0) {
                P.g1 = T.pair_g1[p]; P.g2 = T.pair_g2[p];
                P.b1 = T.geom_bodyid[P.g1]; P.b2 = T.geom_bodyid[P.g2];
            }
            const int g1 = P.g1, g2 = P.g2, b1 = P.b1, b2 = P.b2;
            double pq[4], gq[4], xq[4], R[9], t[3], gp[3], ce[3];
            for (int k = 0; k < 4; k++) { gq[k] = mb[A.o.geom_quat + 4 * g1 + k]; xq[k] = S[L.xquat + 4 * b1 + k]; }
            quat_mul(pq, xq, gq);
            quat_to_mat(R, pq);
            double m1[9], m2[9];
            for (int k = 0; k < 9; k++) { m1[k] = S[L.xmat + 9 * b1 + k]; m2[k] = S[L.xmat + 9 * b2 + k]; }
            for (int k = 0; k < 3; k++) { gp[k] = mb[A.o.geom_pos + 3 * g1 + k]; ce[k] = mb[A.o.geom_center + 3 * g2 + k]; }
            mat_vec(t, m1, gp);
            double ppos[3], n[3] = {R[2], R[5], R[8]};
            for (int k = 0; k < 3; k++) ppos[k] = S[L.xpos + 3 * b1 + k] + t[k];
            mat_vec(t, m2, ce);
            double cd = 0;
            for (int k = 0; k < 3; k++) cd += n[k] * (S[L.xpos + 3 * b2 + k] + t[k] - ppos[k]);
            const double margin = fmax(mb[A.o.geom_margin + g1], mb[A.o.geom_margin + g2]);
            keep = !(cd - mb[A.o.geom_rbound + g2] > margin);
        }
        unsigned long long mask = __ballot(keep);
        while (mask) {
            const int pi = p0 + __ffsll((long long)mask) - 1;
            mask &= mask - 1;
            const PairConst P = pair_of(T, PC, pi);
            const int g1 = P.g1, g2 = P.g2, b1 = P.b1, b2 = P.b2;
            double pq[4], gq[4], xq[4], R[9], t[3], gp[3], m1[9], m2[9], xp2[3];
            for (int k = 0; k < 4; k++) { gq[k] = mb[A.o.geom_quat + 4 * g1 + k]; xq[k] = S[L.xquat + 4 * b1 + k]; }
            quat_mul(pq, xq, gq);
            quat_to_mat(R, pq);
            for (int k = 0; k < 9; k++) { m1[k] = S[L.xmat + 9 * b1 + k]; m2[k] = S[L.xmat + 9 * b2 + k]; }
            for (int k = 0; k < 3; k++) { gp[k] = mb[A.o.geom_pos + 3 * g1 + k]; xp2[k] = S[L.xpos + 3 * b2 + k]; }
            mat_vec(t, m1, gp);
            double ppos[3], n[3] = {R[2], R[5], R[8]};
            for (int k = 0; k < 3; k++) ppos[k] = S[L.xpos + 3 * b1 + k] + t[k];
            const double margin = fmax(mb[A.o.geom_margin + g1], mb[A.o.geom_margin + g2]);
            const double gap = fmax(mb[A.o.geom_gap + g1], mb[A.o.geom_gap + g2]);
            const double rr = mb[A.o.geom_radius + g2];
            const int va = P.va, vn = P.vn;
            double bd = 1e300;
            int bv = 0x7fffffff;
            for (int v = va + LANE; v < va + vn; v += UHC_WAVE) {
                double lv[3] = {mb[A.o.mesh_vert + 3 * v], mb[A.o.mesh_vert + 3 * v + 1], mb[A.o.mesh_vert + 3 * v + 2]}, w[3];
                mat_vec(w, m2, lv);
                double dist = 0;
                for (int k = 0; k < 3; k++) dist += n[k] * (w[k] + xp2[k] - ppos[k]);
                if (dist < bd) { bd = dist; bv = v; }
            }
            {
                const double mn = wave_min(bd);
                const unsigned long long tie = __builtin_amdgcn_ballot_w64(bd == mn);
                int cand = bd == mn ? bv : 0x7fffffff;
                if (__popcll(tie) == 1) cand = __builtin_amdgcn_readlane(bv, __ffsll((long long)tie) - 1);
                else {
#pragma unroll
                    for (int o = 32; o > 0; o >>= 1) cand = min(cand, __shfl_xor(cand, o));
                }
                bd = mn; bv = cand;
            }
            bd -= rr;
            if (bd > margin || bv == 0x7fffffff) continue;
            double cax[3] = {0, 0, 0};
            const bool capsule = (P.dim & 256) != 0;
            if (capsule) {
                double dl[3];
                for (int k = 0; k < 3; k++) dl[k] = mb[A.o.mesh_vert + 3 * va + k] - mb[A.o.mesh_vert + 3 * (va + 1) + k];
                mat_vec(cax, m2, dl);
            }
            const int* adj = (const int*)(mb + A.o.mesh_adj) + (size_t)bv * A.adjdeg;
            bool ok = false;
            double w[3] = {0, 0, 0}, dist = 0;
            const int v = LANE == 0 ? bv : (LANE <= A.adjdeg ? adj[LANE - 1] : -1);
            if (v >= 0) {
// ... 13 lines not shown
            const int want = ncon + min((int)__popcll(cm), T.plane_mesh_maxcon);
            if (want > cap_of<TIER>(A).maxcon) *overflow |= (hands_on<TIER>(A) ? 1 : 2) | UHC_WHY_CONTACTS;
            ncon = min(cap_of<TIER>(A).maxcon, want);
        }
    }
    PROF(32)
    if constexpr (DENSE) {
        int* cand = (int*)(S + L.rowMisc);
        constexpr int CAND_CAP = 256;
        int ncand = 0;
        for (int p0 = 0; p0 < T.ncpair; p0 += UHC_WAVE) {
            const int p = p0 + LANE;
            bool c = false;
            if (p < T.ncpair) {
                const int g1 = T.cpair_g1[p], g2 = T.cpair_g2[p], b1 = T.geom_bodyid[g1], b2 = T.geom_bodyid[g2];
                double ce1[3], ce2[3], t1[3], t2[3], R1[9], R2[9];
                for (int k = 0; k < 9; k++) { R1[k] = S[L.xmat + 9 * b1 + k]; R2[k] = S[L.xmat + 9 * b2 + k]; }
                for (int k = 0; k < 3; k++) { ce1[k] = mb[A.o.geom_center + 3 * g1 + k]; ce2[k] = mb[A.o.geom_center + 3 * g2 + k]; }
                mat_vec(t1, R1, ce1); mat_vec(t2, R2, ce2);
                double d2 = 0;
                for (int k = 0; k < 3; k++) { const double d = (t1[k] + S[L.xpos + 3 * b1 + k]) - (t2[k] + S[L.xpos + 3 * b2 + k]); d2 += d * d; }
                const double margin = fmax(mb[A.o.geom_margin + g1], mb[A.o.geom_margin + g2]);
                const double bound = mb[A.o.geom_rbound + g1] + mb[A.o.geom_rbound + g2] + margin;
                c = !(d2 > bound * bound);
                if (c && !(A.dbg & 128)) {
                    const double* B1 = mb + A.o.geom_box + 6 * g1;
                    const double* B2 = mb + A.o.geom_box + 6 * g2;
                    double c1[3], c2[3], dw[3];
                    mat_vec(c1, R1, B1); mat_vec(c2, R2, B2);
                    for (int k = 0; k < 3; k++) dw[k] = (c2[k] + S[L.xpos + 3 * b2 + k]) - (c1[k] + S[L.xpos + 3 * b1 + k]);
                    double C[3][3], ta[3], tb[3];
                    for (int i = 0; i < 3; i++) {
                        ta[i] = dw[0] * R1[i] + dw[1] * R1[3 + i] + dw[2] * R1[6 + i];
                        tb[i] = dw[0] * R2[i] + dw[1] * R2[3 + i] + dw[2] * R2[6 + i];
                        for (int k = 0; k < 3; k++) C[i][k] = fabs(R1[i] * R2[k] + R1[3 + i] * R2[3 + k] + R1[6 + i] * R2[6 + k]);
                    }
                    bool apart = false;
                    for (int i = 0; i < 3; i++) {
                        apart |= fabs(ta[i]) > B1[3 + i] + B2[3] * C[i][0] + B2[4] * C[i][1] + B2[5] * C[i][2] + margin;
                        apart |= fabs(tb[i]) > B2[3 + i] + B1[3] * C[0][i] + B1[4] * C[1][i] + B1[5] * C[2][i] + margin;
                    }
                    c = !apart;
                }
            }
            const unsigned long long cm = __ballot(c);
            const int rank = ncand + __popcll(cm & ((1ull << LANE) - 1ull));
            if (c && rank < CAND_CAP) cand[rank] = p;
            ncand += (int)__popcll(cm);
        }
        if (ncand > CAND_CAP) { *overflow |= (hands_on<TIER>(A) ? 1 : 2) | UHC_WHY_CANDIDATES; ncand = CAND_CAP; }
        PROF(33)
        const int vstage = cap_of<TIER>(A).vstage;
        if (vstage >= 0 && ncand > 0)
            for (int i = LANE; i < 3 * T.nmeshvert; i += UHC_WAVE) S[vstage + i] = mb[A.o.mesh_vert + i];
        wsync();
        PROF(34)
        for (int c0 = 0; c0 < ncand; c0 += UHC_WAVE) {
            const int ci = c0 + LANE;
            const bool act = ci < ncand;
            int g1 = 0, g2 = 0;
            double gap = 0;
            MprLane M;
            M.b1 = M.b2 = M.voff1 = M.vn1 = M.voff2 = M.vn2 = 0;
            M.hm1 = M.hm2 = 0; M.c1 = M.c2 = v3(0, 0, 0);
            double margin = 0;
            if (act) {
                const int p = cand[ci];
                g1 = T.cpair_g1[p]; g2 = T.cpair_g2[p];
                M.b1 = T.geom_bodyid[g1]; M.b2 = T.geom_bodyid[g2];
                M.voff1 = 3 * T.geom_vertadr[g1]; M.vn1 = T.geom_vertnum[g1];
                M.voff2 = 3 * T.geom_vertadr[g2]; M.vn2 = T.geom_vertnum[g2];
                double ce1[3], ce2[3], t1[3], t2[3], R1[9], R2[9];
                for (int k = 0; k < 9; k++) { R1[k] = S[L.xmat + 9 * M.b1 + k]; R2[k] = S[L.xmat + 9 * M.b2 + k]; }
                for (int k = 0; k < 3; k++) { ce1[k] = mb[A.o.geom_center + 3 * g1 + k]; ce2[k] = mb[A.o.geom_center + 3 * g2 + k]; }
                mat_vec(t1, R1, ce1); mat_vec(t2, R2, ce2);
                M.c1 = v3(t1[0] + S[L.xpos + 3 * M.b1], t1[1] + S[L.xpos + 3 * M.b1 + 1], t1[2] + S[L.xpos + 3 * M.b1 + 2]);
                M.c2 = v3(t2[0] + S[L.xpos + 3 * M.b2], t2[1] + S[L.xpos + 3 * M.b2 + 1], t2[2] + S[L.xpos + 3 * M.b2 + 2]);
                margin = fmax(mb[A.o.geom_margin + g1], mb[A.o.geom_margin + g2]);
                M.hm1 = 0.5 * margin + mb[A.o.geom_radius + g1]; M.hm2 = 0.5 * margin + mb[A.o.geom_radius + g2];
                gap = fmax(mb[A.o.geom_gap + g1], mb[A.o.geom_gap + g2]);
            }
#if defined(UHC_NW2)
            if constexpr (TIER == 2) {
                if (vstage >= 0) mpr_wave_mw<true>(S + vstage, S + L.xmat, S + L.xpos, act, M, mpr_mb<TIER>(A, S), vstage, mb + A.o.mesh_vert);
                else mpr_wave_mw<false>(mb + A.o.mesh_vert, S + L.xmat, S + L.xpos, act, M, mpr_mb<TIER>(A, S), -1, mb + A.o.mesh_vert);
            } else
#endif
            if (vstage >= 0) mpr_wave(S + vstage, S + L.xmat, S + L.xpos, act, M);
            else mpr_wave(mb + A.o.mesh_vert, S + L.xmat, S + L.xpos, act, M);
            const bool hit = act && M.hit && !(M.dir.x == 0 && M.dir.y == 0 && M.dir.z == 0);
            const unsigned long long hm = __ballot(hit);
            const int rank = __popcll(hm & ((1ull << LANE) - 1ull));
            if (hit && ncon + rank < cap_of<TIER>(A).maxcon) {
                const double cp[3] = {M.pos.x, M.pos.y, M.pos.z}, nn[3] = {M.dir.x, M.dir.y, M.dir.z};
                k_write_contact<TIER>(A, mb, S, ncon + rank, g1, g2, M.b1, M.b2, max(T.geom_condim[g1], T.geom_condim[g2]), cp, nn, margin - M.depth, margin, gap);
            }
            const int want = ncon + (int)__popcll(hm);
            if (want > cap_of<TIER>(A).maxcon) *overflow |= (hands_on<TIER>(A) ? 1 : 2) | UHC_WHY_CONTACTS;
            ncon = min(cap_of<TIER>(A).maxcon, want);
        }
        PROF(35)
    }
    wsync();
    return ncon;
}

#define ROW_FRICTION 1
#define ROW_LIMIT 2
#define ROW_CONTACT 3
#define ROW_PYR 4
#define ROW_TWO 0x10
#define ROW_NEG 0x20
#define RTYPE(t) ((t) & 0xf)
struct RowMisc { int type, last, aux, edge; };

template <int TIER, bool DENSE>
__device__ __forceinline__ int k_enumerate_rows(const KernelArgs& A, const double* mb, double* S, int ncon, int* overflow) {
    const DevTopo& T = A.t;
    const DevLds& L = lds_of<TIER>(A);
    RowMisc* RM = (RowMisc*)(S + L.rowMisc);
    int nefc = 0;
    for (int i0 = 0; i0 < T.nv; i0 += UHC_WAVE) {
        const int i = i0 + LANE;
        const bool has = i < T.nv && mb[A.o.dof_frictionloss + i] > 0;
        const unsigned long long m = __ballot(has);
        const int r = nefc + __popcll(m & ((1ull << LANE) - 1ull));
        if (has && r < cap_of<TIER>(A).maxefc) { RM[r].type = ROW_FRICTION; RM[r].last = i; RM[r].aux = i; RM[r].edge = 1; }
        nefc += __popcll(m);
    }
    for (int j0 = 0; j0 < T.njnt; j0 += UHC_WAVE) {
        const int j = j0 + LANE;
        bool lo = false, hi = false, ball = false;
        if (j < T.njnt && T.jnt_limited[j]) {
            const int jt = T.jnt_type[j];
            if (jt == UHC_JNT_HINGE || jt == UHC_JNT_SLIDE) {
                const double v = S[L.qpos + T.jnt_qposadr[j]], mg = mb[A.o.jnt_margin + j];
                lo = (v - mb[A.o.jnt_range + 2 * j]) < mg;
                hi = (mb[A.o.jnt_range + 2 * j + 1] - v) < mg;
            } else if (DENSE && jt == UHC_JNT_BALL) {
                double jac[3];
                ball = true;
                lo = ball_limit(S + L.qpos + T.jnt_qposadr[j], mb + A.o.jnt_range + 2 * j, jac) < mb[A.o.jnt_margin + j];
            }
        }
        const unsigned long long ml = __ballot(lo), mh = __ballot(hi), below = (1ull << LANE) - 1ull;
        int r = nefc + __popcll(ml & below) + __popcll(mh & below);
        if (lo) { if (r < cap_of<TIER>(A).maxefc) { RM[r].type = ROW_LIMIT; RM[r].last = T.jnt_dofadr[j] + (ball ? 2 : 0); RM[r].aux = j; RM[r].edge = ball ? 2 : -1; } r++; }
        if (hi) { if (r < cap_of<TIER>(A).maxefc) { RM[r].type = ROW_LIMIT; RM[r].last = T.jnt_dofadr[j]; RM[r].aux = j; RM[r].edge = 1; } }
        nefc += __popcll(ml) + __popcll(mh);
    }
    wsync();
    if (LANE == 0) {
        int r = nefc, trunc = 0, ntwo = 0, twofull = 0;
        int* NI = (int*)(S + L.ncon_nefc);
        const int maxtwo = !DENSE ? 0 : cap_of<TIER>(A).ndense;
        for (int c = 0; c < ncon; c++) {
            const double* C = S + L.con + c * UHC_CON_STRIDE;
            if (C[12] >= C[13]) continue;
            const int dim = (int)C[21], b1 = (int)C[19], b2 = (int)C[20];
            const int nr = dim == 1 ? 1 : 4, l1 = T.body_lastdof[b1], l2 = T.body_lastdof[b2];
            const bool two = DENSE && l1 >= 0 && l2 >= 0;
            if (TIER == 1 && A.truncate && r + nr > cap_of<TIER>(A).maxefc) { trunc = 1; break; }
            if (two && ntwo + nr > maxtwo) { twofull = 1; if (hands_on<TIER>(A)) break; continue; }
            for (int e = 0; e < nr; e++, r++)
                if (r < cap_of<TIER>(A).maxefc) {
                    int ty = dim == 1 ? ROW_CONTACT : ROW_PYR;
                    if (two) { ty |= ROW_TWO | (ntwo << 8); NI[4 + ntwo] = r; ntwo++; }
                    else if (l2 < 0) ty |= ROW_NEG;
// ... 1096 lines not shown
                        if (LC.v0) zfix[LANE] += fk * Dk[LANE];
                        if (LC.v1) zfix[LANE + UHC_WAVE] += fk * Dk[LANE + UHC_WAVE];
                    }
                    wsync();
                }
                if (valid) {
                    double yb = 0.0;
                    if (two) {
                        const double* D = S + L.dense + row.two * A.nvp;
                        for (int i = 0; i < T.nv; i++) yb = fma(D[i], zfix[i], yb);
                    } else {
                        const short* anc = T.dof_anc + rm.last * YS;
                        const double* Yr = S + L.Y + row.yoff;
                        for (int k = 0; k < row.len; k++) yb = fma(Yr[k], zfix[anc[k]], yb);
                    }
                    row.b += yb;
                }
            }
            PROF(30)
            const int it = k_pgs_fast<TIER, DENSE>(A, mb, S, nC, row, Y, LC, SLg, nslot PROF_PASS);
            if (it < 0) return -4;
            iters += it > 0 ? it : 1;
            if (block) {
                for (int i = LANE; i < T.nv; i += UHC_WAVE) z[i] += zfix[i];
                wsync();
            }
#pragma unroll
            for (int h = 0; h < NRL; h++) if (in[h] && !fx[h]) S[L.rowF + rr[h]] = 0.0;
            wsync();
            if (valid) S[L.rowF + r] = row.f;
            wsync();
            bool viol[NRL], keep[NRL], anyv = false;
#pragma unroll
            for (int h = 0; h < NRL; h++) {
                viol[h] = keep[h] = false;
                if (!in[h]) continue;
                if (c[h]) { keep[h] = S[L.rowF + rr[h]] > 0.0; continue; }
                const RowMisc q = RM[rr[h]];
                double y = S[L.rowB + rr[h]];
                if (q.type & ROW_TWO) {
                    const double* D = S + L.dense + (q.type >> 8) * A.nvp;
                    for (int i = 0; i < T.nv; i++) y = fma(D[i], z[i], y);
                } else {
                    const int len = T.dof_depth[q.last] + 1;
                    const short* anc = T.dof_anc + q.last * YS;
                    const double* Yr = S + L.Y + RY[rr[h]];
                    for (int k = 0; k < len; k++) y = fma(Yr[k], z[anc[k]], y);
                }
                if (fx[h]) y = fma(S[L.rowR + rr[h]], S[L.rowF + rr[h]], y);
                viol[h] = fx[h] ? fabs(y) > tol : y < -tol;
                anyv = anyv || viol[h];
            }
            PROF(31)
            if (!wave_or(anyv)) {
                for (int i = LANE; i < T.nv; i += UHC_WAVE) ztot[i] += z[i];
                wsync();
                done = true;
            } else {
#pragma unroll
                for (int h = 0; h < NRL; h++) { c[h] = keep[h] || viol[h] || fx[h]; p[h] = keep[h] || fx[h]; }
                wsync();
            }
        }
        if (split) { todo |= G; nomerge = true; continue; }
        if (!done) return -3;
    }
    for (int i = LANE; i < T.nv; i += UHC_WAVE) z[i] = ztot[i];
    wsync();
    return iters | (windowed ? UHC_WS_WINDOWED : 0);
}

template <int TIER>
__device__ __forceinline__ int k_primal(const KernelArgs& A, const double* mb, double* S, int nefc, const LaneConst& LC, const double* Yb, const double* Db, int* nact PROF_ARGS);
#ifdef UHC_WITH_TIER4
#include "uhc_primal.h"
#endif

struct FwdOut { int ncon, nefc, iters, overflow, nact, ytot; };
#define UHC_POISON_BITS 0x7ff8dead7fffbeefll
template <int TIER>
__device__ __forceinline__ void guard_arm(const KernelArgs& A, double* S) {
#ifdef UHC_GUARD_LDS
    if (!A.guard_tab) return;
    const int* g = A.guard_tab + 64 * (TIER - 1);
    wsync();
    if (LANE < g[1]) { S[g[32 + LANE]] = __longlong_as_double(UHC_POISON_BITS); S[g[32 + LANE] + 1] = __longlong_as_double(UHC_POISON_BITS); }
    wsync();
#endif
}
template <int TIER>
__device__ __forceinline__ void guard_check(const KernelArgs& A, const double* S, int env, int kind) {
#ifdef UHC_GUARD_LDS
    if (!A.guard_tab) return;
    const int* g = A.guard_tab + 64 * (TIER - 1);
    const int* o = g + (kind ? 32 : 2);
    wsync();
    if (LANE < g[kind]) {
        if (__double_as_longlong(S[o[LANE]]) != UHC_POISON_BITS || __double_as_longlong(S[o[LANE] + 1]) != UHC_POISON_BITS) {
            if (atomicAdd(A.guard_hits, 1) == 0) { A.guard_hits[1] = (TIER << 16) | (kind << 8) | LANE; A.guard_hits[2] = env; A.guard_hits[3] = o[LANE]; }
        }
    }
#endif
}

template <int TIER, bool DENSE>
__device__ __forceinline__ FwdOut k_forward(const KernelArgs& A, const double* mb, double* S, const LaneConst& LC, const BodyConst& BC, const PairConst& PC, MPark& MP, const int env PROF_ARGS) {
    const DevTopo& T = A.t;
    const DevLds& L = lds_of<TIER>(A);
    FwdOut out = {0, 0, 0, 0, 0, 0};
    k_kinematics<TIER>(A, mb, S, BC PROF_PASS);
    PROF(1)
    k_com_pos<TIER>(A, mb, S, BC);
    PROF(2)
    k_crb<TIER, DENSE>(A, mb, S, MP, BC PROF_PASS);
    PROF(3)
    k_factor<TIER>(A, S, L.LD, LC);
    PROF(4)
    k_com_vel<TIER>(A, S, BC);
    PROF(5)
    k_rne<TIER>(A, S, BC PROF_PASS);
    PROF(6)
    k_smooth<TIER>(A, mb, S, LC);
    PROF(7)
    guard_arm<TIER>(A, S);
    out.ncon = k_collision<TIER, DENSE>(A, mb, S, &out.overflow, PC PROF_PASS);
    PROF(8)
    out.nefc = k_enumerate_rows<TIER, DENSE>(A, mb, S, out.ncon, &out.overflow);
    DofVec x = {0.0, 0.0};
    if (out.overflow & 1) return out;
    if (out.nefc > 0) {
        if constexpr (TIER == 1) {
            FastRow row;
            double Yreg[UHC_YM];
            const int st = k_rows_fast<DENSE>(A, mb, S, out.nefc, row, Yreg, LC, &out.ytot);
            out.overflow |= st | (st == 1 ? UHC_WHY_ROW_STORAGE : 0);
            if (st == 1) return out;
            PROF(9)
            const int* NI = (const int*)(S + L.ncon_nefc);
            out.iters = k_pgs_fast<1, DENSE>(A, mb, S, out.nefc, row, Yreg, LC, NI + 4, DENSE ? NI[2] : 0 PROF_PASS);
            PROF(12)
        } else {
            double* Yb = y_store<TIER>(A, S, env);
            double* Db = d_store<TIER>(A, S, env);
            if (k_rows<TIER>(A, mb, S, out.nefc, LC, Yb, Db)) { out.overflow |= 1 | UHC_WHY_ROW_STORAGE; return out; }
            PROF(9)
            int it = -1;
            if constexpr (TIER == 4) {
                bool fric = false;
                for (int r = LANE; r < out.nefc; r += UHC_WAVE) fric = fric || RTYPE(((const RowMisc*)(S + L.rowMisc))[r].type) == ROW_FRICTION;
                fric = wave_or(fric);
                if (T.solver == 1 && !fric) {
                    it = k_primal<TIER>(A, mb, S, out.nefc, LC, Yb, Db, &out.nact PROF_PASS);
                    out.overflow |= 128;
                    if (it < 0) { out.overflow |= 256; it = -it; }
                } else {
                    if (T.solver == 1) out.overflow |= 4 | 8;
                    it = k_pgs<TIER>(A, mb, S, out.nefc, T.iterations, Yb, Db);
                }
                out.iters = it;
                PROF(11)
            } else {
            const bool lost = T.solver == 1 && (out.overflow & 2) != 0;
            if (T.solver == 1) it = k_as_general<TIER, DENSE>(A, mb, S, out.nefc, LC, lost PROF_PASS);
            if (it >= 0 && (it & UHC_WS_WINDOWED)) { it &= UHC_WS_WINDOWED - 1; out.overflow |= 16; }
            if (it < -1 && T.solver == 1 && A.last_tier == 4) {
                out.overflow |= 1 | UHC_WHY_SOLVER;
                return out;
            }
            if (it < 0) {
                if (T.solver == 1) {
                    for (int r = LANE; r < out.nefc; r += UHC_WAVE) S[L.rowF + r] = S[L.rowW + r];
                    wsync();
                }
                out.overflow |= 4 | ((T.solver == 1 && it != -2) ? (4 << (-it)) : 0);
                it = k_pgs<TIER>(A, mb, S, out.nefc, lost ? min(T.iterations, UHC_LOST_SWEEPS) : T.iterations, Yb, Db);
            }
            out.iters = it;
            PROF(11)
            }
        }
        if (LANE < T.nv) x.a = S[L.z + LANE] * S[L.sdinv + LANE];
        if (LANE + UHC_WAVE < T.nv) x.b = S[L.z + LANE + UHC_WAVE] * S[L.sdinv + LANE + UHC_WAVE];
        k_solve<TIER>(A, S, L.LD, x, 1, LC);
    }
    if (LANE < T.nv) S[L.qacc + LANE] = S[L.smooth + LANE] + x.a;
    if (LANE + UHC_WAVE < T.nv) S[L.qacc + LANE + UHC_WAVE] = S[L.smooth + LANE + UHC_WAVE] + x.b;
    wsync();
    return out;
}

template <int TIER>
__device__ __forceinline__ void k_euler(const KernelArgs& A, double* S, int acc) {
    const DevTopo& T = A.t;
    const DevLds& L = lds_of<TIER>(A);
    const double h = T.timestep;
    for (int i = LANE; i < T.nv; i += UHC_WAVE) S[L.qvel + i] += h * S[acc + i];
    wsync();
    for (int j = LANE; j < T.njnt; j += UHC_WAVE) {
        int qa = T.jnt_qposadr[j], da = T.jnt_dofadr[j];
        const int jt = T.jnt_type[j];
        if (jt == UHC_JNT_FREE) {
            for (int k = 0; k < 3; k++) S[L.qpos + qa + k] += h * S[L.qvel + da + k];
            qa += 3; da += 3;
        }
        if (jt == UHC_JNT_FREE || jt == UHC_JNT_BALL) {
            double w[3] = {S[L.qvel + da], S[L.qvel + da + 1], S[L.qvel + da + 2]}, qr[4], q[4];
            const double n = sqrt(dot3(w, w));
            if (n < UHC_MINVAL) { w[0] = 1; w[1] = w[2] = 0; } else { w[0] /= n; w[1] /= n; w[2] /= n; }
// ... 447 lines not shown
        if (wall_clock64() - t0 > 5000000ull) { if (!quiet) atomicAdd(A.s.q_abort + (f == 0 ? 0 : 1), 1); return -1; }
        __builtin_amdgcn_s_sleep(64);
    }
}
__device__ __forceinline__ int chunk_wait(const KernelArgs& A, const int env, const int c) {
    unsigned long long t0 = wall_clock64();
    const unsigned long long t_in = t0;
    int r, late = 0;
    for (;;) {
        int v = __hip_atomic_load(A.chunk_done + env, __ATOMIC_ACQUIRE, __HIP_MEMORY_SCOPE_AGENT);
        if ((v & 0xffff) == UHC_CHUNK_ALL || (v & UHC_CHUNK_TAKEN)) { r = 0; break; }
        if ((v & 0xffff) >= c) { r = 1; break; }
        if (wall_clock64() - t0 > 5000000ull) {
            if (!(v & UHC_CHUNK_CLOSING) && !(v & UHC_CHUNK_ABANDON) &&
                !__hip_atomic_compare_exchange_strong(A.chunk_done + env, &v, v | UHC_CHUNK_ABANDON, __ATOMIC_ACQ_REL, __ATOMIC_RELAXED, __HIP_MEMORY_SCOPE_AGENT)) continue;
            if ((v & UHC_CHUNK_CLOSING) && !late) { late = 1; t0 = wall_clock64(); continue; }
            atomicAdd(A.s.q_abort, 1);
            r = 0;
            break;
        }
        __builtin_amdgcn_s_sleep(32);
    }
#ifndef UHC_STAGE_PROF
    if (A.dbg & 16) A.s.prof[(size_t)env * UHC_NPROF + 24] += (long long)(wall_clock64() - t_in);
#endif
    return r;
}
template <int MODE, int TIER, bool DENSE>
__global__ void __launch_bounds__(UHC_WAVE) uhc_step_kernel(KernelArgs A, const double* __restrict__ d_action,
                                                            const double* __restrict__ d_tbase, const int* __restrict__ d_active) {
    int place = (int)blockIdx.x, c = 0;
    if constexpr (MODE == 0 && TIER == 1) {
        if (A.chunk > 0) {
            int tk = 0;
            if (LANE == 0) tk = atomicAdd(A.ticket, 1);
            tk = __builtin_amdgcn_readfirstlane(tk);
            c = tk / A.n_env;
            place = tk - c * A.n_env;
        }
    }
    const int env = (A.order && place < A.n_env) ? A.order[place] : place;
    bool go = env >= 0 && env < A.n_env && !(d_active && !d_active[env]);
    if (go && A.tier_want) {
        const int t = A.s.tier_now[env];
        go = t == A.tier_want || !((A.sticky_mask >> t) & 1);
    }
    if constexpr (MODE == 0 && TIER == 1) {
        if (go && c > 0) {
            int w = 0;
            if (LANE == 0) w = chunk_wait(A, env, c);
            w = __builtin_amdgcn_readfirstlane(w);
            go = w != 0;
            __builtin_amdgcn_fence(__ATOMIC_ACQUIRE, "agent");
        }
        if (go) {
            const int lo = A.chunk > 0 ? c * A.chunk : 0, hi = A.chunk > 0 ? lo + A.chunk : 0x7fffffff;
            const int r = uhc_step_env<MODE, TIER, DENSE>(A, d_action, d_tbase, env, lo, hi);
            if (A.chunk > 0) {
                __threadfence();
                if (LANE == 0) __hip_atomic_store(A.chunk_done + env, r == 2 ? c + 1 : UHC_CHUNK_ALL, __ATOMIC_RELEASE, __HIP_MEMORY_SCOPE_AGENT);
            }
        }
        if (A.fin && LANE == 0) { __threadfence(); atomicAdd(A.fin, 1); }
        return;
    }
    if (go) {
#ifdef UHC_WITH_TIER4
        if constexpr (TIER == 3 && MODE != 2) {
            int handed = (A.last_tier == 4 && d_active == A.s.pend3 && A.s.pend3[env] == 2) ? 1 : 0;
            if (!handed) handed = uhc_step_env<MODE, TIER, DENSE>(A, d_action, d_tbase, env);
            if (handed && A.last_tier == 4) {
                wsync();
                __builtin_amdgcn_fence(__ATOMIC_ACQUIRE, "agent");
                uhc_step_env<MODE, 4, true>(A, d_action, d_tbase, env);
            }
        } else uhc_step_env<MODE, TIER, DENSE>(A, d_action, d_tbase, env);
#else
        uhc_step_env<MODE, TIER, DENSE>(A, d_action, d_tbase, env);
#endif
    }
    if (A.fin && LANE == 0) { __threadfence(); atomicAdd(A.fin, 1); }
}
#define UHC_QUEUE_THREADS (UHC_WAVE * UHC_NWG)
template <int MODE, int TIER, bool DENSE>
__global__ void __launch_bounds__(UHC_QUEUE_THREADS) uhc_step_queue_kernel(KernelArgs A, const double* __restrict__ d_action, const double* __restrict__ d_tbase) {
#if defined(UHC_NW4)
    static_assert(TIER == 4, "the four-wave form is tier 4's");
    if (threadIdx.x >= UHC_WAVE) { primal_helper<TIER>(A, smem); return; }
#elif defined(UHC_NW2)
    static_assert(TIER == 2, "the two-wave form is the general tier's");
    if (threadIdx.x >= UHC_WAVE) { mpr_helper<TIER>(A, smem); return; }
#endif
    if (A.started && LANE == 0) atomicAdd(A.started, 1);
    long long* tr = (TIER < 4 && (A.dbg & 16) && (int)blockIdx.x < A.n_env) ? A.s.prof + (size_t)blockIdx.x * UHC_NPROF + 8 + 4 * (TIER - 2) : nullptr;
    if (tr && LANE == 0) { tr[0] = (long long)wall_clock64(); tr[1] = 0; tr[3] = 0; }
    int role = 0;
    for (;;) {
        int env = -1;
        if (LANE == 0) env = queue_claim(A, role, TIER == 4);
        env = __builtin_amdgcn_readfirstlane(env);
        if (env < 0) break;
        if (tr && LANE == 0) { if (tr[1] == 0) tr[1] = (long long)wall_clock64(); tr[3]++; }
        uhc_step_env<MODE, TIER, DENSE>(A, d_action, d_tbase, env);
        wsync();
    }
    if (tr && LANE == 0) tr[2] = (long long)wall_clock64();
    if (A.fin && LANE == 0) { __threadfence(); atomicAdd(A.fin, 1); }
#if defined(UHC_NW4)
    primal_release_helpers<TIER>(A, smem);
#elif defined(UHC_NW2)
    mpr_release_helpers<TIER>(A, smem);
#endif
}
```

### uhc_amd/csrc/uhc_plan.cpp

```cpp
#include "uhc_plan.h"

#include <algorithm>
#include <cstdarg>
#include <cstdio>
#include <cstdlib>
#include <cstring>

static int refuse(std::string* err, const char* fmt, ...) {
    char buf[1024];
    va_list ap;
    va_start(ap, fmt);
    vsnprintf(buf, sizeof buf, fmt, ap);
    va_end(ap);
    *err = buf;
    return 1;
}

BatchKnobs read_knobs() {
    BatchKnobs k;
    auto is = [](const char* name, char c) { const char* e = getenv(name); return e && e[0] == c; };
    auto at_least = [](const char* name, int lo, int* v) { if (const char* e = getenv(name)) *v = std::max(lo, atoi(e)); };
    k.guard = is("UHC_GUARD_LDS", '2') ? 2 : is("UHC_GUARD_LDS", '1') ? 1 : 0;
    if (const char* dbg = getenv("UHC_DEBUG")) k.dbg = atoi(dbg);
    if (k.guard) k.dbg |= 2;
#ifndef UHC_EXPERIMENTS
    k.dbg &= ~0x1f00;
#endif
    if (const char* m = getenv("UHC_TIER_MARKS")) sscanf(m, "%d,%d,%d,%d,%d,%d,%d,%d", k.marks, k.marks + 1, k.marks + 2, k.marks + 3, k.marks + 4, k.marks + 5, k.marks + 6, k.marks + 7);
    if (const char* fd = getenv("UHC_FAST_DENSE")) k.fast_dense_got = sscanf(fd, "%d,%d,%d", &k.fast_dense_kib, &k.fast_dense_rows, &k.fast_dense_con);
    k.fast_dcol_own = is("UHC_FAST_DCOL_OWN", '1');
    if (const char* pad = getenv("UHC_LDS_PAD_FAST")) { k.lds_pad_fast = true; k.lds_pad_fast_kib = atoi(pad); }
    k.force_general = is("UHC_FORCE_GENERAL", '1');
    k.tiers = is("UHC_TIERS", '2') ? 2 : is("UHC_TIERS", '3') ? 3 : 0;
    at_least("UHC_Q2_DIV", 1, &k.q2_div); at_least("UHC_Q2_WAIT", 1, &k.q2_wait_min); at_least("UHC_Q2_MAX", 16, &k.q2_max);
    at_least("UHC_Q3_MAX", 2, &k.q3_max); at_least("UHC_Q4_MAX", 0, &k.q4_max); at_least("UHC_T4_ROWS", 0, &k.t4_rows);
    if (const char* fc = getenv("UHC_FAST_CHUNK")) {
        char* end = nullptr;
        const long v = strtol(fc, &end, 10);
        if (end == fc || *end != 0 || v < 0) k.fast_chunk_bad = true;
        else k.fast_chunk = (v == 0 || v > 0x7fff) ? 0x7fff : (int)v;
    }
    return k;
}

static bool same_topology(const UhcModelDesc& a, const UhcModelDesc& b) {
    if (a.nq != b.nq || a.nv != b.nv || a.nu != b.nu || a.nbody != b.nbody || a.njnt != b.njnt || a.ngeom != b.ngeom ||
        a.nmeshvert != b.nmeshvert || a.nexclude != b.nexclude)
        return false;
    auto eq = [](const int32_t* x, const int32_t* y, size_t n) { return !memcmp(x, y, n * 4); };
    return eq(a.body_parentid, b.body_parentid, a.nbody) && eq(a.jnt_type, b.jnt_type, a.njnt) &&
           eq(a.jnt_bodyid, b.jnt_bodyid, a.njnt) && eq(a.dof_parentid, b.dof_parentid, a.nv) &&
           eq(a.geom_type, b.geom_type, a.ngeom) && eq(a.geom_bodyid, b.geom_bodyid, a.ngeom) &&
           eq(a.geom_vertadr, b.geom_vertadr, a.ngeom) && eq(a.geom_vertnum, b.geom_vertnum, a.ngeom) &&
           eq(a.geom_contype, b.geom_contype, a.ngeom) && eq(a.geom_conaffinity, b.geom_conaffinity, a.ngeom) &&
           eq(a.jnt_limited, b.jnt_limited, a.njnt) && eq(a.geom_condim, b.geom_condim, a.ngeom);
}

static void build_blob(const UhcModelDesc& d, DevNumOff& o, std::vector<double>& blob, int adjdeg) {
    blob.clear();
    auto put = [&](const double* p, size_t n) { int off = (int)blob.size(); blob.insert(blob.end(), p, p + n); return off; };
    o.body_pos = put(d.body_pos, 3 * d.nbody); o.body_quat = put(d.body_quat, 4 * d.nbody);
    o.body_ipos = put(d.body_ipos, 3 * d.nbody); o.body_iquat = put(d.body_iquat, 4 * d.nbody);
    o.body_mass = put(d.body_mass, d.nbody); o.body_inertia = put(d.body_inertia, 3 * d.nbody);
    o.body_invweight0 = put(d.body_invweight0, 2 * d.nbody);
    o.jnt_pos = put(d.jnt_pos, 3 * d.njnt); o.jnt_axis = put(d.jnt_axis, 3 * d.njnt); o.jnt_range = put(d.jnt_range, 2 * d.njnt);
    o.jnt_stiffness = put(d.jnt_stiffness, d.njnt); o.jnt_margin = put(d.jnt_margin, d.njnt);
    o.qpos0 = put(d.qpos0, d.nq); o.qpos_spring = put(d.qpos_spring, d.nq);
    o.dof_armature = put(d.dof_armature, d.nv); o.dof_damping = put(d.dof_damping, d.nv);
    o.dof_frictionloss = put(d.dof_frictionloss, d.nv); o.dof_invweight0 = put(d.dof_invweight0, d.nv);
    o.geom_pos = put(d.geom_pos, 3 * d.ngeom); o.geom_quat = put(d.geom_quat, 4 * d.ngeom);
    o.geom_friction = put(d.geom_friction, 3 * d.ngeom); o.geom_margin = put(d.geom_margin, d.ngeom);
    o.geom_gap = put(d.geom_gap, d.ngeom); o.geom_solref = put(d.geom_solref, 2 * d.ngeom);
    o.geom_solimp = put(d.geom_solimp, 5 * d.ngeom); o.geom_rbound = put(d.geom_rbound, d.ngeom);
    o.geom_center = put(d.geom_center, 3 * d.ngeom);
    o.mesh_vert = put(d.mesh_vert, 3 * (size_t)d.nmeshvert);
    {
        std::vector<double> box((size_t)6 * std::max(d.ngeom, 1), 0.0);
        for (int g = 0; g < d.ngeom; g++) {
            double lo[3] = {1e300, 1e300, 1e300}, hi[3] = {-1e300, -1e300, -1e300};
            const int v0 = d.geom_vertadr ? d.geom_vertadr[g] : 0, nvt = d.geom_vertnum ? d.geom_vertnum[g] : 0;
            for (int v = v0; v < v0 + nvt; v++)
                for (int k = 0; k < 3; k++) { lo[k] = std::min(lo[k], d.mesh_vert[3 * v + k]); hi[k] = std::max(hi[k], d.mesh_vert[3 * v + k]); }
            const double rr = (d.geom_type[g] == UHC_GEOM_SPHERE || d.geom_type[g] == UHC_GEOM_CAPSULE) ? d.geom_size[3 * g] : 0.0;
            for (int k = 0; k < 3; k++) {
                if (nvt > 0) { box[6 * g + k] = 0.5 * (lo[k] + hi[k]); box[6 * g + 3 + k] = 0.5 * (hi[k] - lo[k]) + rr; }
                else { box[6 * g + k] = d.geom_center[3 * g + k]; box[6 * g + 3 + k] = d.geom_rbound[g]; }
            }
        }
        o.geom_box = put(box.data(), box.size());
        std::vector<double> rad((size_t)std::max(d.ngeom, 1), 0.0);
        for (int g = 0; g < d.ngeom; g++)
            if (d.geom_type[g] == UHC_GEOM_SPHERE || d.geom_type[g] == UHC_GEOM_CAPSULE) rad[g] = d.geom_size[3 * g];
        o.geom_radius = put(rad.data(), rad.size());
    }
    o.actuator_gear = put(d.actuator_gear, 3 * (size_t)d.nu);
    o.meaninertia = put(&d.meaninertia, 1);
    {
        std::vector<int32_t> adj((size_t)std::max(d.nmeshvert, 1) * adjdeg + 2, -1);
        for (int v = 0; v < d.nmeshvert; v++)
            for (int e = d.mesh_adjadr[v], k = 0; e < d.mesh_adjadr[v + 1]; e++, k++) adj[(size_t)v * adjdeg + k] = d.mesh_adj[e];
        std::vector<double> packed((adj.size() + 1) / 2, 0.0);
        memcpy(packed.data(), adj.data(), adj.size() / 2 * 2 * sizeof(int32_t));
        o.mesh_adj = put(packed.data(), packed.size());
    }
    while (blob.size() % 2) blob.push_back(0.0);
    o.stride = (int)blob.size();
}

static int validate(const UhcModel* const* models, int n_models, const int32_t* env_model, int n_env, const UhcCtrlDesc* ctrl, int* n_trail_out, std::string* err) {
    if (!models || n_models < 1 || n_env < 1 || !ctrl) return refuse(err, "uhc_batch_create: bad argument");
    const UhcModelDesc& d = models[0]->d;
    for (int k = 1; k < n_models; k++)
        if (!same_topology(d, models[k]->d)) return refuse(err, "uhc_batch_create: model %d differs in topology from model 0", k);
    if (env_model)
        for (int e = 0; e < n_env; e++)
// ... 143 lines not shown
    void end_guard() { if (guard_on) { phase2.push_back(off); off += 2; } }
};
static void common_layout(Carver& cv, const UhcModelDesc& d, const DevTopo& T, DevLds& F, bool fast) {
    const int nv = d.nv, nb = d.nbody, nj = d.njnt;
    cv.off = 0;
    cv.persist.clear(); cv.phase2.clear(); cv.rec = &cv.persist;
    F.qpos = cv.carve(d.nq); F.qvel = cv.carve(nv); F.qacc = cv.carve(nv); F.ctrl = cv.carve(d.nu); F.applied = cv.carve(nv);
    F.bias = cv.carve(nv); F.smooth = cv.carve(nv); F.z = cv.carve(nv); F.dinv = cv.carve(nv); F.sdinv = cv.carve(nv);
    F.zero = cv.carve(2);
    F.mij = fast ? cv.carve((T.nM + 3) / 4 + 1) : 0;
    F.LD = cv.carve(T.nM + 2); F.M = F.LD;
    F.cdof = cv.carve(6 * nv);
    F.xpos = cv.carve(3 * nb); F.xquat = cv.carve(4 * nb); F.xmat = cv.carve(9 * nb); F.xipos = cv.carve(3 * nb); F.rootcom = cv.carve(3 * nb);
    F.vec = fast ? F.z : cv.carve(nv);
    const int base = cv.off;
    cv.rec = nullptr;
    F.cinert = cv.carve(10 * nb);
    const int r2 = cv.off;
    F.ximat = cv.carve(9 * nb); F.xanchor = cv.carve(3 * nj); F.xaxis = cv.carve(3 * nj);
    const int endA = cv.off;
    cv.off = r2;
    F.cdofdot = cv.carve(6 * nv);
    const int r3 = cv.off;
    F.crb = cv.carve(10 * nb);
    const int endB = cv.off;
    cv.off = r3;
    F.cvel = cv.carve(6 * nb); F.cacc = cv.carve(6 * nb); F.cfrc = cv.carve(6 * nb);
    cv.end1 = std::max(std::max(endA, endB), cv.off);
    cv.off = base;
    cv.rec = &cv.phase2;
}

static void fast_layout(Carver& cv, const UhcModelDesc& d, int n_env, const BatchKnobs& knobs, BatchPlan& P) {
    KernelArgs& A = P.A;
    const DevTopo& T = A.t;
    DevLds& F = A.lf;
    const int YS = T.maxdepth + 1;
    common_layout(cv, d, T, F, T.ncpair == 0);
    int dense_kib = 52, fast_maxcon = UHC_FAST_MAXCON, fast_ndense = UHC_FAST_MAXTWO;
    if (T.ncpair > 0) fast_maxcon = UHC_FAST_MAXCON_DENSE;
    bool hinge_only = P.n_trailing_free == 0;
    for (int j = 0; j < d.njnt; j++) hinge_only = hinge_only && d.jnt_type[j] != UHC_JNT_BALL;
    if (T.ncpair > 0 && n_env >= 3072 && hinge_only) { dense_kib = 40; fast_ndense = 6; }
    bool any_ball = false;
    for (int j = 0; j < d.njnt; j++) any_ball = any_ball || d.jnt_type[j] == UHC_JNT_BALL;
    if (T.ncpair > 0 && any_ball && dense_kib == 52) fast_ndense = 9;
    {
        const int got = knobs.fast_dense_got, kib = knobs.fast_dense_kib, nd = knobs.fast_dense_rows, nc = knobs.fast_dense_con;
        if (got >= 2 && kib >= 32 && kib <= 160 && nd >= (T.ncpair > 0 ? 1 : 0) && nd <= UHC_FAST_MAXTWO) { dense_kib = kib; fast_ndense = nd; }
        if (got == 3 && nc >= 8 && nc <= UHC_GEN_MAXCON && T.ncpair > 0) fast_maxcon = nc;
    }
    F.con = cv.carve(fast_maxcon * UHC_CON_STRIDE);
    F.rowMisc = cv.carve(UHC_WAVE * 2);
    F.ncon_nefc = cv.carve(2 + UHC_MAXTWO / 2);
    A.cf.maxefc = UHC_FAST_MAXEFC; A.cf.maxcon = fast_maxcon; A.cf.ld_delta = 0;
    A.cf.ndense = T.ncpair > 0 ? fast_ndense : 0;
    F.dense = cv.carve(A.cf.ndense * A.nvp);
    const bool dcol_alias = A.cf.ndense * UHC_WAVE <= fast_maxcon * UHC_CON_STRIDE && !knobs.fast_dcol_own;
    F.dcol = dcol_alias ? F.con : cv.carve(A.cf.ndense * UHC_WAVE);
    F.Y = cv.off;
    const int budget = T.ncpair > 0 ? (dense_kib * 1024) / 8 : 40 * 1024 / 8;
    int ycap = budget - cv.off - (cv.guard_on ? 2 : 0);
    const int need1 = cv.end1 - cv.off;
    if (ycap < need1) ycap = need1;
    if (ycap < 8 * YS) ycap = 8 * YS;
    A.cf.ycap = ycap;
    A.cf.vstage = ((A.dbg & 2) == 0 && T.ncpair > 0 && 3 * d.nmeshvert <= A.cf.ndense * A.nvp + (dcol_alias ? 0 : A.cf.ndense * UHC_WAVE) + ycap) ? F.dense : -1;
    cv.off += ycap;
    cv.end_guard();
    F.rowR = F.rowAref = F.rowB = F.rowF = F.rowDa = F.rowW = F.rowY = F.dsc = F.Y;
    F.total = cv.off;
    if (A.marks[2] < 0) {
        A.marks[2] = A.cf.ndense > 0 ? A.cf.ndense : UHC_FAST_MAXTWO; A.marks[5] = A.cf.ndense > 0 ? std::max(1, A.cf.ndense - (A.cf.ndense > 8 ? 2 : 1)) : 10;
        A.marks[1] = A.cf.maxcon; A.marks[4] = A.cf.maxcon - std::max(2, A.cf.maxcon / 8);
    }
    P.lds_bytes_fast = (size_t)cv.off * sizeof(double);
    if (knobs.lds_pad_fast) {
        const size_t want = (size_t)knobs.lds_pad_fast_kib * 1024;
        if (want > P.lds_bytes_fast && want <= 160 * 1024) P.lds_bytes_fast = want;
    }
    P.use_fast = !knobs.force_general && P.lds_bytes_fast <= 160 * 1024;
}

static bool rows_layout(Carver& cv, const UhcModelDesc& d, const KernelArgs& A, DevLds& F, TierCap& cp, int maxefc, int maxcon, int maxtwo, int budget_doubles, bool full_y) {
    const DevTopo& T = A.t;
    const int YS = T.maxdepth + 1;
    common_layout(cv, d, T, F, false);
    cp.maxefc = maxefc; cp.maxcon = maxcon; cp.ndense = T.ncpair > 0 ? maxtwo : 0;
    cp.ld_delta = (F.LD - A.lf.LD) * 8;
    F.con = cv.carve(std::max(maxcon * UHC_CON_STRIDE, cp.ndense * UHC_WAVE));
    F.dcol = F.con;
    F.rowMisc = cv.carve(maxefc * 2);
    F.ncon_nefc = cv.carve(2 + UHC_MAXTWO);
    F.rowY = cv.carve(maxefc / 2 + 1);
    F.rowR = cv.carve(maxefc); F.rowAref = cv.carve(maxefc); F.rowB = cv.carve(maxefc); F.rowF = cv.carve(maxefc); F.rowDa = cv.carve(maxefc); F.rowW = cv.carve(maxefc);
    F.dense = cv.carve(cp.ndense * A.nvp);
    F.dsc = cv.carve(cp.ndense * 4);
    F.Y = cv.off;
    const int full = maxefc * YS + 8;
    int ycap = full_y ? full : std::min(budget_doubles - cv.off - (cv.guard_on ? 2 : 0), full);
    if (!full_y && ycap < 64 * 18) return false;
    if (ycap < cv.end1 - cv.off) ycap = cv.end1 - cv.off;
    cp.ycap = ycap & ~1;
    cp.vstage = ((A.dbg & 2) == 0 && T.ncpair > 0 && 3 * d.nmeshvert <= cp.ndense * A.nvp + cp.ndense * 4 + cp.ycap) ? F.dense : -1;
    cv.off += cp.ycap;
    cv.end_guard();
    F.total = cv.off;
    return cv.off <= budget_doubles;
}

static bool huge_layout(Carver& cv, const UhcModelDesc& d, const KernelArgs& A, DevLds& F, TierCap& cp, int maxefc, int maxcon) {
    const DevTopo& T = A.t;
    const int nv = d.nv, YS = T.maxdepth + 1;
    common_layout(cv, d, T, F, false);
    cp.maxefc = maxefc; cp.maxcon = maxcon; cp.ndense = T.ncpair > 0 ? UHC_HUGE_MAXTWO : 0;
    cp.ld_delta = (F.LD - A.lf.LD) * 8;
    const int scratch4 = primal_scratch(nv, YS).total;
    F.con = cv.carve(std::max(cp.maxcon * UHC_CON_STRIDE, scratch4));
    F.dcol = F.con;
    F.rowMisc = cv.carve(std::max(maxefc * 2, 128));
    F.ncon_nefc = cv.carve(2 + (cp.ndense + 1) / 2 + 1);
    F.rowY = cv.carve(maxefc / 2 + 1);
    F.rowR = cv.carve(maxefc); F.rowAref = cv.carve(maxefc); F.rowB = cv.carve(maxefc); F.rowF = cv.carve(maxefc); F.rowDa = cv.carve(maxefc); F.rowW = cv.carve(maxefc);
    F.dsc = cv.carve(std::max(cp.ndense * 4, 2));
    F.H = cv.carve((nv * (nv + 1)) / 2);
    F.Y = F.dense = F.H;
    cp.ycap = maxefc * YS + 8;
    cp.vstage = ((A.dbg & 2) == 0 && T.ncpair > 0 && 3 * d.nmeshvert <= (nv * (nv + 1)) / 2) ? F.H : -1;
    if (cv.off < cv.end1) cv.off = cv.end1;
    cv.end_guard();
    F.total = cv.off;
    return cv.off <= 160 * 1024 / 8;
}

static int upper_tiers(Carver* cv, const UhcModelDesc& d, const BatchKnobs& knobs, BatchPlan& P, std::string* err) {
    KernelArgs& A = P.A;
    A.last_tier = knobs.tiers == 2 ? 2 : 3;
    if (A.last_tier == 3) {
        bool ok = false;
        for (int me = UHC_BIG_MAXEFC; me > UHC_GEN_MAXEFC && !ok; me -= 32) {
            ok = rows_layout(cv[2], d, A, A.lh, A.ch, me, me / 2, UHC_BIG_MAXTWO, 160 * 1024 / 8, true);
        }
        if (ok) P.lds_bytes_big = (size_t)A.lh.total * sizeof(double);
        else A.last_tier = 2;
    }
    const int two_per_cu = 79 * 1024 / 8;
    bool ok = A.last_tier == 3 && rows_layout(cv[1], d, A, A.l, A.cg, UHC_GEN_MAXEFC, UHC_GEN_MAXCON, UHC_GEN_MAXTWO, two_per_cu, false);
    if (!ok) {
        if (!rows_layout(cv[1], d, A, A.l, A.cg, UHC_GEN_MAXEFC, UHC_GEN_MAXCON, A.last_tier == 2 ? UHC_MAXTWO : UHC_GEN_MAXTWO, 160 * 1024 / 8, true))
            return refuse(err, "uhc_batch_create: model needs %zu B of LDS per env (> 160 KiB)", (size_t)A.l.total * 8);
    }
    P.lds_bytes = (size_t)A.l.total * sizeof(double);
    A.lx = A.lh; A.cx = A.ch; A.gY = A.gD = nullptr; A.gy_stride = A.gd_stride = 0;
    if (A.last_tier == 3 && knobs.tiers != 3) {
        bool ok4 = false;
        int best_me = 0, best_mc = 0;
        double best = -1.0;
        for (int me = UHC_HUGE_MAXEFC; me >= 384; me -= 128) {
            if (!huge_layout(cv[3], d, A, A.lx, A.cx, me, UHC_HUGE_MAXCON)) continue;
            int mc = UHC_HUGE_MAXCON_MOST;
            while (mc > UHC_HUGE_MAXCON && !huge_layout(cv[3], d, A, A.lx, A.cx, me, mc)) mc -= 8;
            const double score = std::min(me / 2.75, (double)mc);
            if (score > best) { best = score; best_me = me; best_mc = mc; }
        }
        ok4 = best_me > 0 && huge_layout(cv[3], d, A, A.lx, A.cx, best_me, best_mc);
        if (ok4 && (A.dbg & 64)) fprintf(stderr, "uhc tier 4: %d rows / %d contacts / %d body-body rows, %d B of LDS\n", A.cx.maxefc, A.cx.maxcon, A.cx.ndense, A.lx.total * 8);
        if (ok4) {
            A.last_tier = 4;
            P.lds_bytes_big = std::max(P.lds_bytes_big, (size_t)A.lx.total * sizeof(double));
            A.gy_stride = A.cx.ycap;
            A.gd_stride = std::max(A.cx.ndense, 1) * A.nvp;
        } else { A.lx = A.lh; A.cx = A.ch; }
    }
    return 0;
}

static int guard_table(Carver* cv, const BatchKnobs& knobs, BatchPlan& P, std::string* err) {
    P.guard_tab.assign(4 * 64, 0);
    if (knobs.guard == 2) cv[0].persist.push_back(P.A.lf.qpos);
    for (int t = 0; t < 4; t++) {
        if (cv[t].persist.size() > 30 || cv[t].phase2.size() > 32) return refuse(err, "uhc_batch_create: UHC_GUARD_LDS: more guard words than the table holds");
        P.guard_tab[64 * t] = (int)cv[t].persist.size(); P.guard_tab[64 * t + 1] = (int)cv[t].phase2.size();
        for (size_t k = 0; k < cv[t].persist.size(); k++) P.guard_tab[64 * t + 2 + k] = cv[t].persist[k];
        for (size_t k = 0; k < cv[t].phase2.size(); k++) P.guard_tab[64 * t + 32 + k] = cv[t].phase2[k];
    }
    return 0;
}

static int schedules(const UhcModelDesc& d, BatchPlan& P, std::string* err) {
    KernelArgs& A = P.A;
    DevTopo& T = A.t;
    const int nv = d.nv, YS = T.maxdepth + 1;
    const std::vector<int>& dof_depth = P.dof_depth;
    const size_t sol_steps = (size_t)((std::max(nv - 1, 1) + 7) / 8 * 8 + 8);
    std::vector<unsigned int>& fac_prog = P.fac_prog;
    P.sol_back.assign(sol_steps * 64, 0); P.sol_fwd.assign(sol_steps * 64, 0);
    const unsigned ldb = (unsigned)A.lf.LD * 8u;
    auto adr = [&](int rel) { return ldb + 8u * (unsigned)rel; };
    const int ZERO = T.nM, DUMP = T.nM + 1;
    if (adr(DUMP) + 8 > 65536u || (unsigned)A.l.LD * 8u + 8u * (T.nM + 2) > 65536u) return refuse(err, "uhc_batch_create: LD buffer beyond the 16-bit schedule addresses");
    int ngroups = 0;
    for (int k = nv - 1; k >= 1; k--) {
        const int dk = dof_depth[k], kk = d.dof_madr[k];
        if (!dk) continue;
        std::vector<unsigned> E;
        int anc = k;
        for (int a = 1; a <= dk; a++) {
            anc = d.dof_parentid[anc];
            for (int t = 0; t <= dk - a; t++) { E.push_back(adr(kk + a) | (adr(kk + a + t) << 16)); E.push_back(adr(d.dof_madr[anc] + t)); }
        }
        constexpr int G = 3;
        while ((E.size() / 2) % (64 * G)) { E.push_back(adr(ZERO) | (adr(ZERO) << 16)); E.push_back(adr(DUMP)); }
        const int ng = (int)(E.size() / 2 / (64 * G));
        for (int gi = 0; gi < ng; gi++)
            for (int l = 0; l < 64; l++) {
                size_t e[G];
                for (int q = 0; q < G; q++) e[q] = ((size_t)gi * 64 * G + 64 * q + l) * 2;
                const unsigned nr = (gi == ng - 1 && l < dk) ? adr(kk + 1 + l) : adr(ZERO);
                for (int q = 0; q < G; q++) fac_prog.push_back(E[e[q]]);
                fac_prog.push_back(E[e[0] + 1] | (E[e[1] + 1] << 16));
                fac_prog.push_back(E[e[2] + 1] | (nr << 16));
                fac_prog.push_back(adr(kk));
            }
        ngroups += ng;
    }
    T.fac_nslot = ngroups;
    for (int q = 0; q < 2 * 64; q++) {
        for (int w = 0; w < 3; w++) fac_prog.push_back(adr(ZERO) | (adr(ZERO) << 16));
        fac_prog.push_back(adr(DUMP) | (adr(DUMP) << 16)); fac_prog.push_back(adr(DUMP) | (adr(ZERO) << 16)); fac_prog.push_back(adr(ZERO));
    }
    auto entry = [&](int i, int j) -> unsigned {
        if (i >= nv || j >= nv || j >= i || dof_depth[j] >= dof_depth[i]) return adr(ZERO);
        return P.dof_anc[(size_t)i * YS + dof_depth[j]] == j ? adr(d.dof_madr[i] + dof_depth[i] - dof_depth[j]) : adr(ZERO);
    };
    for (size_t q = 0; q < sol_steps * 64; q++) P.sol_back[q] = P.sol_fwd[q] = adr(ZERO) | (adr(ZERO) << 16);
// ... 29 lines not shown

#define PLAN_TRY(x) do { if (x) return 1; } while (0)
int plan_batch(const UhcModel* const* models, int n_models, const int32_t* env_model, int n_env, const UhcCtrlDesc* ctrl, const BatchKnobs& knobs,
               BatchPlan* out, std::string* err) {
    BatchPlan& P = *out;
    P = BatchPlan();
    if (knobs.fast_chunk_bad) return refuse(err, "uhc_batch_create: UHC_FAST_CHUNK must be a non-negative integer (substeps per chunk of the fast tier's control step)");
    PLAN_TRY(validate(models, n_models, env_model, n_env, ctrl, &P.n_trailing_free, err));
    const UhcModelDesc& d = models[0]->d;
    KernelArgs& A = P.A;
    memset(&A, 0, sizeof A);
    DevTopo& T = A.t;
    const int nv = d.nv;
    T.nq = d.nq; T.nv = nv; T.nu = d.nu; T.nbody = d.nbody; T.njnt = d.njnt; T.ngeom = d.ngeom; T.nmeshvert = d.nmeshvert;
    T.nM = d.dof_madr[nv];
    T.iterations = d.iterations; T.plane_mesh_maxcon = d.plane_mesh_maxcon; T.solver = d.solver;
    T.timestep = d.timestep; T.tolerance = d.tolerance;
    for (int k = 0; k < 3; k++) T.gravity[k] = d.gravity[k];
    T.has_damping = 0;
    for (int k = 0; k < n_models; k++)
        for (int i = 0; i < nv; i++) T.has_damping |= models[k]->d.dof_damping[i] > 0;
    for (int j = 0; j < d.njnt; j++) A.ball_limits |= d.jnt_type[j] == UHC_JNT_BALL && d.jnt_limited[j] != 0;
    A.n_env = n_env;
    tree_tables(d, P);
    PLAN_TRY(validate_trees(d, P, err));
    PLAN_TRY(collision_pairs(d, P, err));
    PLAN_TRY(model_blobs(models, n_models, P, err));
    PLAN_TRY(controller(d, ctrl, P, err));
    if (T.nM > 64 * 24) return refuse(err, "uhc_batch_create: nM %d > 1536 (the register tile that carries M between substeps)", T.nM);
    A.nvp = (nv + 1) & ~1;
    A.dbg = knobs.dbg;
    A.t4_rows = knobs.t4_rows;
    for (int k = 0; k < 8; k++) A.marks[k] = knobs.marks[k];
    Carver cv[4];
    for (Carver& c : cv) c.guard_on = knobs.guard != 0;
    fast_layout(cv[0], d, n_env, knobs, P);
    PLAN_TRY(upper_tiers(cv, d, knobs, P, err));
    if (knobs.guard) PLAN_TRY(guard_table(cv, knobs, P, err));
    PLAN_TRY(schedules(d, P, err));
    PLAN_TRY(actuator_table(d, P, err));
    return 0;
}

FastChunks plan_fast_chunks(int n_substeps, int chunk, int n_env) {
    FastChunks f;
    f.chunk = (chunk <= 0 || chunk >= n_substeps) ? 0 : chunk;
    f.n_chunks = f.chunk ? (n_substeps + f.chunk - 1) / f.chunk : 1;
    f.grid = f.n_chunks * n_env;
    f.prod_total = f.grid;
    return f;
}
void fast_chunk_range(const FastChunks& f, int n_substeps, int c, int* lo, int* hi) {
    *lo = f.chunk ? c * f.chunk : 0;
    *hi = f.chunk ? std::min(*lo + f.chunk, n_substeps) : n_substeps;
}
#define UHC_FAST_CHUNK_DEFAULT 5
int default_fast_chunk(int knob, int n_substeps, int n_env, int n_cu, size_t lds_bytes_fast) {
    if (knob > 0) return knob >= n_substeps ? 0 : knob;
    const int per_cu = std::max(1, std::min(4, (int)(160 * 1024 / std::max<size_t>(lds_bytes_fast, 1))));
    return (n_env > per_cu * n_cu && UHC_FAST_CHUNK_DEFAULT < n_substeps) ? UHC_FAST_CHUNK_DEFAULT : 0;
}

StickySizes plan_sticky_step(const StickyInputs& in) {
    StickySizes s;
    s.fast = plan_fast_chunks(in.n_substeps, in.n_substeps > 0 ? default_fast_chunk(in.fast_chunk, in.n_substeps, in.n_env, in.n_cu, in.lds_bytes_fast) : 0, in.n_env);
    const int est2 = in.est2, est3 = in.est3, est4 = in.est4, n_env = in.n_env, n_cu = in.n_cu;
    const bool big = in.last_tier >= 3;
    s.launch4 = in.last_tier == 4 && est4 > 0 && in.est2_then > 0 && big && !in.queues_off;
    s.queues = est2 > 0;
    s.waiting = s.queues && est2 <= (3 * n_env) / 4 && !in.queues_off;
    s.q3 = s.queues && big;
    const int share3 = est3 > 0 ? (int)((2ll * n_cu * est3) / std::max(1, est2 + 2 * est3)) : 0;
    s.grid3 = s.waiting ? std::min(est3 + est3 / 4 + 2, in.q3_max) : std::min(est3 + est3 / 4 + 2, std::max(64, std::min(share3, (3 * n_cu) / 4)));
    const int room2 = 2 * (n_cu - (in.large_first && s.q3 ? std::min(s.grid3, std::max(est3, 1)) : 0));
    const int s1 = std::max(1, std::min(4, (int)(160 * 1024 / std::max<size_t>(in.lds_bytes_fast, 1))));
    const int est1 = std::max(0, n_env - est2 - est3);
    const int bal = (int)(((long long)est2 * s1 * n_cu) / std::max(1, est1 + (est2 * s1) / 2));
    const int cap2 = in.fixed_cap2 ? in.q2_max : std::max(in.q2_max, std::min((7 * bal) / 8, (3 * n_cu) / 2));
    s.grid2 = s.waiting ? std::min(est2 / in.q2_div + 8, cap2) : std::min(est2 + est2 / 4 + 8, std::min(n_env, std::max(64, room2)));
    s.sticky_mask = (s.queues ? 4 : 0) | (s.q3 ? 8 : 0) | (s.launch4 ? 16 : 0);
    s.q4 = s.launch4 && s.q3;
    s.grid4 = std::min(in.q4_max, est4 + est4 / 2 + 2);
    s.n_wait = std::min(64, std::max(in.q2_wait_min, 2 * in.handed2 + 8));
    return s;
}
```

### uhc_amd/csrc/uhc_plan.h

```cpp
#pragma once
#include <string>
#include <vector>

#include "uhc_host.h"

struct BatchKnobs {
    int dbg = 0;
    int marks[8] = {64, 16, -1, 56, 14, 10, 8, 7};
    int fast_dense_got = 0, fast_dense_kib = 0, fast_dense_rows = 0, fast_dense_con = 0;
    bool fast_dcol_own = false;
    bool lds_pad_fast = false;
    int lds_pad_fast_kib = 0;
    bool force_general = false;
    int tiers = 0;
    int guard = 0;
    int q2_div = 1, q2_wait_min = 16, q2_max = 256, q3_max = 32, q4_max = 16;
    int t4_rows = 0;
    int fast_chunk = 0;
    bool fast_chunk_bad = false;
};
BatchKnobs read_knobs();

struct BatchPlan {
    KernelArgs A;
    size_t lds_bytes = 0, lds_bytes_fast = 0, lds_bytes_big = 0;
    bool use_fast = true;
    int n_trailing_free = 0;
    std::vector<int> body_depth, body_rootid, body_nsub, body_lastdof, dof_depth, dof_ndesc, dof_rootid;
    std::vector<short> dof_anc, m_row, m_col;
    std::vector<unsigned short> m_ij;
    std::vector<unsigned char> ncommon;
    std::vector<int> pg1, pg2, cg1, cg2;
    std::vector<double> model_blob;
    std::vector<unsigned int> fac_prog, sol_back, sol_fwd, chain;
    std::vector<int> dof_act;
    std::vector<int> vf_body;
    std::vector<int> guard_tab;
};
int plan_batch(const UhcModel* const* models, int n_models, const int32_t* env_model, int n_env, const UhcCtrlDesc* ctrl, const BatchKnobs& knobs,
               BatchPlan* out, std::string* err);

struct StickyInputs {
    int est2, est3, est4;
    int est2_then;
    int handed2;
    int n_env, n_cu;
    size_t lds_bytes_fast;
    bool large_first;
    int last_tier;
    bool queues_off;
    int q2_div, q2_wait_min, q2_max, q3_max, q4_max;
    bool fixed_cap2;
    int fast_chunk;
    int n_substeps;
};
struct FastChunks {
    int chunk;
    int n_chunks;
    int grid;
    int prod_total;
};
FastChunks plan_fast_chunks(int n_substeps, int chunk, int n_env);
void fast_chunk_range(const FastChunks& f, int n_substeps, int c, int* lo, int* hi);
int default_fast_chunk(int knob, int n_substeps, int n_env, int n_cu, size_t lds_bytes_fast);
struct StickySizes {
    bool queues, waiting, q3, q4, launch4;
    int grid2, grid3, grid4, n_wait, sticky_mask;
    FastChunks fast;
};
StickySizes plan_sticky_step(const StickyInputs& in);
```

Before: 101,800.

## Overlap general-tier collision detection on helper wave with forward dynamics

Adds a new general-tier queue kernel variant in which the helper wave runs collision detection, dispatched through a new MCMD_COLL mailbox command. Meanwhile the main wave computes COM, CRB, mass matrix and smooth forces, then joins to serve the remaining MPR rounds. A separate LDS layout keeps the collision scratch clear of phase-1 data. The path is used only when the queue grids leave enough CUs free, and it costs extra LDS, a new kernel instance and more intricate cross-wave synchronisation.

```diff
diff --git a/__graft_entry__.py b/__graft_entry__.py
--- a/__graft_entry__.py
+++ b/__graft_entry__.py
@@ -5,7 +5,7 @@
 ROOT = os.path.dirname(os.path.abspath(__file__))
 CSRC = os.path.join(ROOT, "uhc_amd", "csrc")
 LIB = os.path.join(CSRC, "libuhc_amd.so")
-HIP_SOURCES = ["uhc_k_fast.hip", "uhc_k_fast_dense.hip", "uhc_k_fast_fwd.hip", "uhc_k_fast_fwd_dense.hip", "uhc_k_general.hip", "uhc_k_general_fwd.hip", "uhc_k_big.hip", "uhc_k_big_fwd.hip", "uhc_k_general_q.hip", "uhc_k_big_q.hip", "uhc_k_huge_q.hip",
+HIP_SOURCES = ["uhc_k_fast.hip", "uhc_k_fast_dense.hip", "uhc_k_fast_fwd.hip", "uhc_k_fast_fwd_dense.hip", "uhc_k_general.hip", "uhc_k_general_fwd.hip", "uhc_k_big.hip", "uhc_k_big_fwd.hip", "uhc_k_general_q.hip", "uhc_k_general_qo.hip", "uhc_k_big_q.hip", "uhc_k_huge_q.hip",
                "uhc_batch_kernels.hip", "uhc_env.hip", "uhc_rollout.hip", "uhc_plan.cpp", "uhc_capi.cpp", "uhc_env_capi.cpp"]
 HIP_HEADERS = ["uhc_physics_impl.h", "uhc_primal.h", "uhc_mpr.h", "uhc_device.h", "uhc_device_env.h", "uhc_host.h", "uhc_plan.h", "uhc_launch.h"]
 
diff --git a/uhc_amd/csrc/uhc_capi.cpp b/uhc_amd/csrc/uhc_capi.cpp
--- a/uhc_amd/csrc/uhc_capi.cpp
+++ b/uhc_amd/csrc/uhc_capi.cpp
@@ -73,6 +73,7 @@
 #ifdef UHC_GUARD_LDS
     f |= 8;
 #endif
+    if (!read_knobs().gen_overlap) f |= 16;
     return f;
 }
 
@@ -189,7 +190,9 @@
     TRY(upload(b, dvec(ctrl->jkp), &A.c.jkp)); TRY(upload(b, dvec(ctrl->jkd), &A.c.jkd));
     TRY(upload(b, dvec(ctrl->torque_lim), &A.c.torque_lim)); TRY(upload(b, dvec(ctrl->a_scale), &A.c.a_scale));
     if (!P.guard_tab.empty()) {
-        const std::vector<int>& tab = P.guard_tab;
+        std::vector<int> tab = P.guard_tab;
+        tab.resize(5 * 64, 0);
+        std::copy(P.guard_tab_ovl.begin(), P.guard_tab_ovl.end(), tab.begin() + 4 * 64);
         int* d_tab = nullptr;
         TRY(dalloc(b, tab.size(), &d_tab)); TRY(dalloc(b, 4, &b->d_guard_hits));
         HIP_OK(hipMemcpy(d_tab, tab.data(), tab.size() * sizeof(int), hipMemcpyHostToDevice));
@@ -263,11 +266,21 @@
     b->nM = P.A.t.nM;
     b->lds_bytes = P.lds_bytes; b->lds_bytes_fast = P.lds_bytes_fast; b->lds_bytes_big = P.lds_bytes_big;
     b->use_fast = P.use_fast;
+#ifdef UHC_STAGE_PROF
+    b->gen_overlap = false;
+#else
+    b->gen_overlap = P.lds_bytes_ovl > 0;
+#endif
+    b->l_ovl = P.l_ovl; b->cg_ovl = P.cg_ovl; b->lds_bytes_ovl = P.lds_bytes_ovl;
+    if (P.A.dbg & 64)
+        fprintf(stderr, "uhc batch: general tier %zu B, overlap layout %s (%zu B; UHC_GEN_OVERLAP %s)\n", b->lds_bytes, b->gen_overlap ? "on" : "off", b->lds_bytes_ovl,
+                knobs.gen_overlap ? "not 0" : "= 0");
     b->hbm_guard = knobs.guard != 0;
     b->q2_div = knobs.q2_div; b->q2_wait_min = knobs.q2_wait_min; b->q2_max = knobs.q2_max; b->q3_max = knobs.q3_max; b->q4_max = knobs.q4_max;
     b->fast_chunk = (P.A.dbg & 4) ? 0x7fff : knobs.fast_chunk;
     TRY(upload_plan(b, P, models[0]->d, ctrl, h_env_model));
     HIP_OK(uhc_set_lds_limit(b->lds_bytes, b->lds_bytes_fast, b->lds_bytes_big));
+    if (b->gen_overlap) HIP_OK(uhc_launch_m0_gen_qo_lds(b->lds_bytes_ovl));
     TRY(alloc_state(b, models, h_env_model));
     HIP_OK(hipStreamCreateWithFlags(&b->own_stream, hipStreamNonBlocking));
     b->stream = b->own_stream;
@@ -378,6 +391,7 @@
     StickyInputs in{};
     in.est4 = est4; in.est2_then = est2_then; in.n_env = b->n_env; in.n_cu = b->n_cu; in.lds_bytes_fast = b->lds_bytes_fast; in.large_first = b->large_first;
     in.fast_chunk = b->fast_chunk; in.n_substeps = b->A.c.n_substeps;
+    in.gen_overlap = b->gen_overlap;
     in.last_tier = b->A.last_tier; in.q2_div = b->q2_div; in.q2_wait_min = b->q2_wait_min; in.q2_max = b->q2_max; in.q3_max = b->q3_max; in.q4_max = b->q4_max;
 #ifdef UHC_EXPERIMENTS
     in.fixed_cap2 = (b->A.dbg & 2048) != 0;
@@ -437,7 +451,15 @@
             K.fin = b->d_fin + 2; K.started = waiting ? b->d_fin + 3 : nullptr;
             K.n_wait = z.n_wait; K.spares = b->d_fin;
             K.q_next = q3 ? b->d_lists + b->n_env : nullptr; K.q_next_count = q3 ? b->d_counts + 3 : nullptr;
-            HIP_OK(uhc_launch_step(mode, 2, &K, d_action, d_tbase, nullptr, b->lds_bytes, b->side_stream));
+            if (z.overlap2) {
+                const DevLds l = K.l; const TierCap cg = K.cg;
+                K.l = b->l_ovl; K.cg = b->cg_ovl; K.gen_overlap = 1;
+                if (b->A.dbg & 64) fprintf(stderr, "uhc step %lld: %d general-tier consumers on the overlap layout (%zu B)\n", b->cnt_step, grid2, b->lds_bytes_ovl);
+                HIP_OK(uhc_launch_m0_gen_qo(&K, d_action, d_tbase, nullptr, b->lds_bytes_ovl, b->side_stream));
+                K.l = l; K.cg = cg; K.gen_overlap = 0;
+            } else {
+                HIP_OK(uhc_launch_step(mode, 2, &K, d_action, d_tbase, nullptr, b->lds_bytes, b->side_stream));
+            }
             HIP_OK(hipEventRecord(b->ev_side1, b->side_stream));
         }
         if (q3 && !b->large_first) { if (launch_large()) return -1; }
diff --git a/uhc_amd/csrc/uhc_device.h b/uhc_amd/csrc/uhc_device.h
--- a/uhc_amd/csrc/uhc_device.h
+++ b/uhc_amd/csrc/uhc_device.h
@@ -182,6 +182,7 @@
     int* ticket;
     int* chunk_done;
     int* chunk_rec;
+    int gen_overlap;
 };
 #define UHC_CHUNK_ALL 0x7fff
 #define UHC_CHUNK_ABANDON (1 << 30)
diff --git a/uhc_amd/csrc/uhc_host.h b/uhc_amd/csrc/uhc_host.h
--- a/uhc_amd/csrc/uhc_host.h
+++ b/uhc_amd/csrc/uhc_host.h
@@ -48,6 +48,10 @@
     int q4_max = 16;
     int q3_max = 32;
     int fast_chunk = 0;
+    bool gen_overlap = false;
+    DevLds l_ovl;
+    TierCap cg_ovl;
+    size_t lds_bytes_ovl = 0;
     int *d_lists = nullptr, *d_counts = nullptr, *d_cursors = nullptr, *d_fin = nullptr;
     bool queues_off = false;
     int* h_counts = nullptr;
diff --git a/uhc_amd/csrc/uhc_k_general_qo.hip b/uhc_amd/csrc/uhc_k_general_qo.hip
--- /dev/null
+++ b/uhc_amd/csrc/uhc_k_general_qo.hip
@@ -0,0 +1,6 @@
+#define UHC_NW2
+#define UHC_GEN_OVL
+#include "uhc_physics_impl.h"
+#include "uhc_launch.h"
+
+UHC_QUEUE_OVL_LAUNCH(m0_gen_qo, UHC_QUEUE_THREADS)
diff --git a/uhc_amd/csrc/uhc_launch.h b/uhc_amd/csrc/uhc_launch.h
--- a/uhc_amd/csrc/uhc_launch.h
+++ b/uhc_amd/csrc/uhc_launch.h
@@ -16,6 +16,7 @@
                                             hipStream_t stream);                                                                                 \
     extern "C" hipError_t uhc_launch_##name##_lds(size_t lds_bytes);
 UHC_STEP_INSTANCES(UHC_DECL_LAUNCH)
+UHC_DECL_LAUNCH(m0_gen_qo, 0, 2, true, true)
 
 #define UHC_DEFINE_LAUNCH(name, KERNEL, MODE, TIER, DENSE, THREADS, GRID, ...)                                                                        \
     extern "C" hipError_t uhc_launch_##name(const KernelArgs* A, const double* d_action, const double* d_tbase, const int* d_active, size_t lds_bytes, \
@@ -30,6 +31,17 @@
 #define UHC_ENV_LAUNCH(name, MODE, TIER, DENSE) UHC_DEFINE_LAUNCH(name, uhc_step_kernel, MODE, TIER, DENSE, UHC_WAVE, A->grid ? A->grid : A->n_env, d_active)
 #define UHC_QUEUE_LAUNCH(name, TIER, THREADS) UHC_DEFINE_LAUNCH(name, uhc_step_queue_kernel, 0, TIER, true, THREADS, A->grid)
 
+#define UHC_QUEUE_OVL_LAUNCH(name, THREADS)                                                                                                          \
+    extern "C" hipError_t uhc_launch_##name(const KernelArgs* A, const double* d_action, const double* d_tbase, const int* d_active, size_t lds_bytes, \
+                                            hipStream_t stream) {                                                                                     \
+        (void)d_active;                                                                                                                               \
+        hipLaunchKernelGGL((uhc_step_queue_kernel<0, 2, true, true>), dim3(A->grid), dim3(THREADS), lds_bytes, stream, *A, d_action, d_tbase);         \
+        return hipGetLastError();                                                                                                                     \
+    }                                                                                                                                                 \
+    extern "C" hipError_t uhc_launch_##name##_lds(size_t lds_bytes) {                                                                                 \
+        return hipFuncSetAttribute((const void*)uhc_step_queue_kernel<0, 2, true, true>, hipFuncAttributeMaxDynamicSharedMemorySize, (int)lds_bytes); \
+    }
+
 struct UhcStepInstance { int mode, tier; bool dense, queue; UhcStepLaunch launch; UhcSetLds set_lds; int lds; };
 #define UHC_INSTANCE_ROW(name, mode, tier, dense, queue) {mode, tier, dense, queue, uhc_launch_##name, uhc_launch_##name##_lds, tier == 1 ? 1 : tier == 2 ? 0 : 2},
 #define UHC_STEP_TABLE {UHC_STEP_INSTANCES(UHC_INSTANCE_ROW)}
diff --git a/uhc_amd/csrc/uhc_mpr.h b/uhc_amd/csrc/uhc_mpr.h
--- a/uhc_amd/csrc/uhc_mpr.h
+++ b/uhc_amd/csrc/uhc_mpr.h
@@ -418,8 +418,10 @@
 }
 
 #if defined(UHC_NW2)
-enum { MCMD_EXIT = 0, MCMD_ROUND = 1, MCMD_ROWS = 2 };
+enum { MCMD_EXIT = 0, MCMD_ROUND = 1, MCMD_ROWS = 2, MCMD_COLL = 3, MCMD_COLL_DONE = 4 };
 struct MprMB { int* hdr; double* io[6]; double* hm1; double* hm2; int* st4; int* st2; };
+static_assert(UHC_GEN_MAXEFC <= 2 * UHC_WAVE && UHC_GEN_MAXEFC >= 128, "the two-wave consumer builds rows 0 .. 127 and lays its mailbox on arrays of 128 doubles");
+static_assert(4 + UHC_WAVE <= UHC_GEN_MAXEFC && 2 * UHC_WAVE <= UHC_GEN_MAXEFC, "mailbox pieces inside rowR .. rowW");
 template <int TIER>
 __device__ __forceinline__ MprMB mpr_mb(const KernelArgs& A, double* S) {
     const DevLds& L = lds_of<TIER>(A);
@@ -474,7 +476,7 @@
         take -= 1;
     }
 }
-template <bool LDSV>
+template <bool LDSV, bool OWN = false>
 __device__ __forceinline__ void mpr_wave_mw(const double* __restrict__ VB, const double* __restrict__ xmat, const double* __restrict__ xpos, bool active, MprLane& M, const MprMB& MB, int vstage,
                                             const double* vb_global) {
     CcdSup p0, p1, p2, p3, v4;
@@ -493,18 +495,26 @@
         MB.hm1[LANE] = M.hm1; MB.hm2[LANE] = M.hm2;
     }
     int* mbi = MB.hdr;
-    if (LANE == 0) {
+    if (!OWN && LANE == 0) {
         mbi[3] = LDSV ? vstage : -1;
         mbi[4] = (int)((unsigned long long)vb_global & 0xffffffffull); mbi[5] = (int)((unsigned long long)vb_global >> 32);
     }
+    int joined = 0;
     for (int round = 0;; round++) {
         const unsigned long long live = __builtin_amdgcn_ballot_w64(st != MPR_DONE);
         if (!live || round == UHC_MPR_MAXSUP) break;
         if (st != MPR_DONE) { MB.io[0][LANE] = dir.x; MB.io[1][LANE] = dir.y; MB.io[2][LANE] = dir.z; }
-        if (LANE == 0) { mbi[0] = MCMD_ROUND; mbi[1] = (int)(live & 0xffffffffull); mbi[2] = (int)(live >> 32); }
-        __syncthreads();
-        mpr_serve_round(VB, xmat, xpos, MB, live, 0, UHC_NWG);
-        __syncthreads();
+        if (OWN && !joined) joined = __builtin_amdgcn_readfirstlane(__hip_atomic_load(mbi + 6, __ATOMIC_RELAXED, __HIP_MEMORY_SCOPE_WORKGROUP));
+        if (OWN && !joined) {
+            wsync();
+            mpr_serve_round(VB, xmat, xpos, MB, live, 0, 1);
+            wsync();
+        } else {
+            if (LANE == 0) { mbi[0] = MCMD_ROUND; mbi[1] = (int)(live & 0xffffffffull); mbi[2] = (int)(live >> 32); }
+            __syncthreads();
+            mpr_serve_round(VB, xmat, xpos, MB, live, OWN ? 1 : 0, UHC_NWG);
+            __syncthreads();
+        }
         if (st != MPR_DONE) { v4.v = v3(MB.io[0][LANE], MB.io[1][LANE], MB.io[2][LANE]); v4.s = v3(MB.io[3][LANE], MB.io[4][LANE], MB.io[5][LANE]); }
         bool to_refine = false, to_pen = false;
         if (st == MPR_D1) {
@@ -583,6 +593,18 @@
         __syncthreads();
         const int cmd = __builtin_amdgcn_readfirstlane(mbi[0]);
         if (cmd == MCMD_EXIT) return;
+#if defined(UHC_GEN_OVL)
+        if (cmd == MCMD_COLL) {
+            const unsigned long long mbp = ((unsigned long long)(unsigned)__builtin_amdgcn_readfirstlane(mbi[5]) << 32) | (unsigned)__builtin_amdgcn_readfirstlane(mbi[4]);
+            int overflow = 0;
+            const PairConst HPC = pair_const(A.t);
+            PROF_DECL
+            const int ncon = k_collision<TIER, true, true>(A, (const double*)mbp, S, &overflow, HPC PROF_PASS);
+            if (LANE == 0) { MB.hdr[0] = MCMD_COLL_DONE; MB.hdr[1] = ncon; MB.hdr[2] = overflow; }
+            __syncthreads();
+            continue;
+        }
+#endif
         if (cmd == MCMD_ROWS) {
             const int nefc = __builtin_amdgcn_readfirstlane(mbi[1]), ntwo = __builtin_amdgcn_readfirstlane(mbi[2]);
             const unsigned long long mbp = ((unsigned long long)(unsigned)__builtin_amdgcn_readfirstlane(mbi[5]) << 32) | (unsigned)__builtin_amdgcn_readfirstlane(mbi[4]);
@@ -604,6 +626,25 @@
     }
 }
 template <int TIER>
+__device__ __forceinline__ int mpr_join(const KernelArgs& A, const double* mb, double* S, int* overflow) {
+    const DevLds& L = lds_of<TIER>(A);
+    const MprMB MB = mpr_mb<TIER>(A, S);
+    int* mbi = MB.hdr;
+    const int vst = cap_of<TIER>(A).vstage;
+    if (LANE == 0) __hip_atomic_store(mbi + 6, 1, __ATOMIC_RELAXED, __HIP_MEMORY_SCOPE_WORKGROUP);
+    for (;;) {
+        __syncthreads();
+        const int cmd = __builtin_amdgcn_readfirstlane(mbi[0]);
+        if (cmd != MCMD_ROUND) break;
+        const unsigned long long live = ((unsigned long long)(unsigned)__builtin_amdgcn_readfirstlane(mbi[2]) << 32) | (unsigned)__builtin_amdgcn_readfirstlane(mbi[1]);
+        if (vst >= 0) mpr_serve_round(S + vst, S + L.xmat, S + L.xpos, MB, live, 0, UHC_NWG);
+        else mpr_serve_round(mb + A.o.mesh_vert, S + L.xmat, S + L.xpos, MB, live, 0, UHC_NWG);
+        __syncthreads();
+    }
+    *overflow |= __builtin_amdgcn_readfirstlane(mbi[2]);
+    return __builtin_amdgcn_readfirstlane(mbi[1]);
+}
+template <int TIER>
 __device__ __forceinline__ void mpr_release_helpers(const KernelArgs& A, double* S) {
     int* mbi = mpr_mb<TIER>(A, S).hdr;
     if (LANE == 0) mbi[0] = MCMD_EXIT;
diff --git a/uhc_amd/csrc/uhc_physics_impl.h b/uhc_amd/csrc/uhc_physics_impl.h
--- a/uhc_amd/csrc/uhc_physics_impl.h
+++ b/uhc_amd/csrc/uhc_physics_impl.h
@@ -91,6 +91,9 @@
 struct LaneConst { int d0, d1, n0, n1, m0, m1, pk0, pk1, r0, r1; bool v0, v1; };
 template <int TIER> __device__ __forceinline__ void k_dense_groups(const KernelArgs& A, double* S, const LaneConst& LC, double* Db, const int ntwo, const int first, const int stride);
 template <bool DENSE> __device__ __forceinline__ LaneConst lane_const(const DevTopo& T);
+struct PairConst { int g1, g2, b1, b2, va, vn, dim; };
+__device__ __forceinline__ PairConst pair_const(const DevTopo& T);
+template <int TIER, bool DENSE, bool HOWN = false> __device__ __forceinline__ int k_collision(const KernelArgs& A, const double* mb, double* S, int* overflow, const PairConst& PC PROF_ARGS);
 #include "uhc_mpr.h"
 
 __device__ __forceinline__ void cross3(double* r, const double* a, const double* b) {
@@ -716,7 +719,6 @@
     else y = 1 - pow((1 - x) / (1 - mid), power) * (1 - mid);
     return dmin + y * (dmax - dmin);
 }
-struct PairConst { int g1, g2, b1, b2, va, vn, dim; };
 __device__ __forceinline__ int pair_dim(const DevTopo& T, int g1, int g2) {
     return max(T.geom_condim[g1], T.geom_condim[g2]) | ((T.geom_type[g2] == UHC_GEOM_CAPSULE && T.geom_vertnum[g2] == 2) ? 256 : 0);
 }
@@ -780,7 +782,7 @@
     for (int k = 0; k < 3; k++) jac[k] = -sg * ax[k];
     return fmax(range[0], range[1]) - value;
 }
-template <int TIER, bool DENSE>
+template <int TIER, bool DENSE, bool HOWN>
 __device__ __forceinline__ int k_collision(const KernelArgs& A, const double* mb, double* S, int* overflow, const PairConst& PC PROF_ARGS) {
     const DevTopo& T = A.t;
     const DevLds& L = lds_of<TIER>(A);
@@ -960,8 +962,8 @@
             }
 #if defined(UHC_NW2)
             if constexpr (TIER == 2) {
-                if (vstage >= 0) mpr_wave_mw<true>(S + vstage, S + L.xmat, S + L.xpos, act, M, mpr_mb<TIER>(A, S), vstage, mb + A.o.mesh_vert);
-                else mpr_wave_mw<false>(mb + A.o.mesh_vert, S + L.xmat, S + L.xpos, act, M, mpr_mb<TIER>(A, S), -1, mb + A.o.mesh_vert);
+                if (vstage >= 0) mpr_wave_mw<true, HOWN>(S + vstage, S + L.xmat, S + L.xpos, act, M, mpr_mb<TIER>(A, S), vstage, mb + A.o.mesh_vert);
+                else mpr_wave_mw<false, HOWN>(mb + A.o.mesh_vert, S + L.xmat, S + L.xpos, act, M, mpr_mb<TIER>(A, S), -1, mb + A.o.mesh_vert);
             } else
 #endif
             if (vstage >= 0) mpr_wave(S + vstage, S + L.xmat, S + L.xpos, act, M);
@@ -2224,7 +2226,7 @@
 __device__ __forceinline__ void guard_arm(const KernelArgs& A, double* S) {
 #ifdef UHC_GUARD_LDS
     if (!A.guard_tab) return;
-    const int* g = A.guard_tab + 64 * (TIER - 1);
+    const int* g = A.guard_tab + 64 * ((TIER == 2 && A.gen_overlap) ? 4 : TIER - 1);
     wsync();
     if (LANE < g[1]) { S[g[32 + LANE]] = __longlong_as_double(UHC_POISON_BITS); S[g[32 + LANE] + 1] = __longlong_as_double(UHC_POISON_BITS); }
     wsync();
@@ -2234,7 +2236,7 @@
 __device__ __forceinline__ void guard_check(const KernelArgs& A, const double* S, int env, int kind) {
 #ifdef UHC_GUARD_LDS
     if (!A.guard_tab) return;
-    const int* g = A.guard_tab + 64 * (TIER - 1);
+    const int* g = A.guard_tab + 64 * ((TIER == 2 && A.gen_overlap) ? 4 : TIER - 1);
     const int* o = g + (kind ? 32 : 2);
     wsync();
     if (LANE < g[kind]) {
@@ -2252,6 +2254,18 @@
     FwdOut out = {0, 0, 0, 0, 0, 0};
     k_kinematics<TIER>(A, mb, S, BC PROF_PASS);
     PROF(1)
+#if defined(UHC_GEN_OVL)
+    constexpr bool ovl = TIER == 2;
+    if (ovl) {
+        guard_arm<TIER>(A, S);
+        int* mbi = mpr_mb<TIER>(A, S).hdr;
+        if (LANE == 0) {
+            mbi[0] = MCMD_COLL; mbi[6] = 0;
+            mbi[4] = (int)((unsigned long long)mb & 0xffffffffull); mbi[5] = (int)((unsigned long long)mb >> 32);
+        }
+        __syncthreads();
+    }
+#endif
     k_com_pos<TIER>(A, mb, S, BC);
     PROF(2)
     k_crb<TIER, DENSE>(A, mb, S, MP, BC PROF_PASS);
@@ -2264,8 +2278,12 @@
     PROF(6)
     k_smooth<TIER>(A, mb, S, LC);
     PROF(7)
+#if defined(UHC_GEN_OVL)
+    out.ncon = mpr_join<TIER>(A, mb, S, &out.overflow);
+#else
     guard_arm<TIER>(A, S);
     out.ncon = k_collision<TIER, DENSE>(A, mb, S, &out.overflow, PC PROF_PASS);
+#endif
     PROF(8)
     out.nefc = k_enumerate_rows<TIER, DENSE>(A, mb, S, out.ncon, &out.overflow);
     DofVec x = {0.0, 0.0};
@@ -2879,13 +2897,18 @@
     if (A.fin && LANE == 0) { __threadfence(); atomicAdd(A.fin, 1); }
 }
 #define UHC_QUEUE_THREADS (UHC_WAVE * UHC_NWG)
-template <int MODE, int TIER, bool DENSE>
+template <int MODE, int TIER, bool DENSE, bool OVL = false>
 __global__ void __launch_bounds__(UHC_QUEUE_THREADS) uhc_step_queue_kernel(KernelArgs A, const double* __restrict__ d_action, const double* __restrict__ d_tbase) {
 #if defined(UHC_NW4)
     static_assert(TIER == 4, "the four-wave form is tier 4's");
     if (threadIdx.x >= UHC_WAVE) { primal_helper<TIER>(A, smem); return; }
 #elif defined(UHC_NW2)
     static_assert(TIER == 2, "the two-wave form is the general tier's");
+#if defined(UHC_GEN_OVL)
+    static_assert(OVL, "this translation unit compiles the overlap order into every k_forward<2, *>");
+#else
+    static_assert(!OVL, "the overlap order is compiled with -DUHC_GEN_OVL (uhc_k_general_qo.hip)");
+#endif
     if (threadIdx.x >= UHC_WAVE) { mpr_helper<TIER>(A, smem); return; }
 #endif
     if (A.started && LANE == 0) atomicAdd(A.started, 1);
diff --git a/uhc_amd/csrc/uhc_plan.cpp b/uhc_amd/csrc/uhc_plan.cpp
--- a/uhc_amd/csrc/uhc_plan.cpp
+++ b/uhc_amd/csrc/uhc_plan.cpp
@@ -31,6 +31,7 @@
     k.fast_dcol_own = is("UHC_FAST_DCOL_OWN", '1');
     if (const char* pad = getenv("UHC_LDS_PAD_FAST")) { k.lds_pad_fast = true; k.lds_pad_fast_kib = atoi(pad); }
     k.force_general = is("UHC_FORCE_GENERAL", '1');
+    k.gen_overlap = !is("UHC_GEN_OVERLAP", '0');
     k.tiers = is("UHC_TIERS", '2') ? 2 : is("UHC_TIERS", '3') ? 3 : 0;
     at_least("UHC_Q2_DIV", 1, &k.q2_div); at_least("UHC_Q2_WAIT", 1, &k.q2_wait_min); at_least("UHC_Q2_MAX", 16, &k.q2_max);
     at_least("UHC_Q3_MAX", 2, &k.q3_max); at_least("UHC_Q4_MAX", 0, &k.q4_max); at_least("UHC_T4_ROWS", 0, &k.t4_rows);
@@ -340,10 +341,12 @@
     P.use_fast = !knobs.force_general && P.lds_bytes_fast <= 160 * 1024;
 }
 
-static bool rows_layout(Carver& cv, const UhcModelDesc& d, const KernelArgs& A, DevLds& F, TierCap& cp, int maxefc, int maxcon, int maxtwo, int budget_doubles, bool full_y) {
+static bool rows_layout(Carver& cv, const UhcModelDesc& d, const KernelArgs& A, DevLds& F, TierCap& cp, int maxefc, int maxcon, int maxtwo, int budget_doubles, bool full_y,
+                        bool overlap = false) {
     const DevTopo& T = A.t;
     const int YS = T.maxdepth + 1;
     common_layout(cv, d, T, F, false);
+    if (overlap) cv.off = cv.end1;
     cp.maxefc = maxefc; cp.maxcon = maxcon; cp.ndense = T.ncpair > 0 ? maxtwo : 0;
     cp.ld_delta = (F.LD - A.lf.LD) * 8;
     F.con = cv.carve(std::max(maxcon * UHC_CON_STRIDE, cp.ndense * UHC_WAVE));
@@ -409,6 +412,26 @@
             return refuse(err, "uhc_batch_create: model needs %zu B of LDS per env (> 160 KiB)", (size_t)A.l.total * 8);
     }
     P.lds_bytes = (size_t)A.l.total * sizeof(double);
+    P.lds_bytes_ovl = 0;
+    if (ok && knobs.gen_overlap) {
+        Carver co;
+        co.guard_on = cv[1].guard_on;
+        const int phase1 = cv[1].end1 - A.l.con;
+        const bool fits = rows_layout(co, d, A, P.l_ovl, P.cg_ovl, UHC_GEN_MAXEFC, UHC_GEN_MAXCON, UHC_GEN_MAXTWO, two_per_cu + phase1, false, true);
+        const TierCap &a = A.cg, &o = P.cg_ovl;
+        const bool same = a.maxefc == o.maxefc && a.maxcon == o.maxcon && a.ndense == o.ndense && a.ycap == o.ycap && a.ld_delta == o.ld_delta && (a.vstage >= 0) == (o.vstage >= 0);
+        if (fits && same && phase1 > 0 && P.l_ovl.con >= co.end1 && (size_t)P.l_ovl.total * sizeof(double) <= 160 * 1024) {
+            P.lds_bytes_ovl = (size_t)P.l_ovl.total * sizeof(double);
+            P.ovl_phase1_end = co.end1;
+            if (co.guard_on) {
+                P.guard_tab_ovl.assign(64, 0);
+                if (co.persist.size() > 30 || co.phase2.size() > 32) return refuse(err, "uhc_batch_create: UHC_GUARD_LDS: more guard words than the table holds");
+                P.guard_tab_ovl[0] = (int)co.persist.size(); P.guard_tab_ovl[1] = (int)co.phase2.size();
+                for (size_t k = 0; k < co.persist.size(); k++) P.guard_tab_ovl[2 + k] = co.persist[k];
+                for (size_t k = 0; k < co.phase2.size(); k++) P.guard_tab_ovl[32 + k] = co.phase2[k];
+            }
+        }
+    }
     A.lx = A.lh; A.cx = A.ch; A.gY = A.gD = nullptr; A.gy_stride = A.gd_stride = 0;
     if (A.last_tier == 3 && knobs.tiers != 3) {
         bool ok4 = false;
@@ -604,5 +627,6 @@
     s.q4 = s.launch4 && s.q3;
     s.grid4 = std::min(in.q4_max, est4 + est4 / 2 + 2);
     s.n_wait = std::min(64, std::max(in.q2_wait_min, 2 * in.handed2 + 8));
+    s.overlap2 = in.gen_overlap && s.queues && 2 * (s.grid2 + (s.q3 ? s.grid3 : 0)) <= n_cu;
     return s;
 }
diff --git a/uhc_amd/csrc/uhc_plan.h b/uhc_amd/csrc/uhc_plan.h
--- a/uhc_amd/csrc/uhc_plan.h
+++ b/uhc_amd/csrc/uhc_plan.h
@@ -18,6 +18,7 @@
     int t4_rows = 0;
     int fast_chunk = 0;
     bool fast_chunk_bad = false;
+    bool gen_overlap = true;
 };
 BatchKnobs read_knobs();
 
@@ -36,6 +37,11 @@
     std::vector<int> dof_act;
     std::vector<int> vf_body;
     std::vector<int> guard_tab;
+    DevLds l_ovl{};
+    TierCap cg_ovl{};
+    size_t lds_bytes_ovl = 0;
+    int ovl_phase1_end = 0;
+    std::vector<int> guard_tab_ovl;
 };
 int plan_batch(const UhcModel* const* models, int n_models, const int32_t* env_model, int n_env, const UhcCtrlDesc* ctrl, const BatchKnobs& knobs,
                BatchPlan* out, std::string* err);
@@ -53,6 +59,7 @@
     bool fixed_cap2;
     int fast_chunk;
     int n_substeps;
+    bool gen_overlap;
 };
 struct FastChunks {
     int chunk;
@@ -67,5 +74,6 @@
     bool queues, waiting, q3, q4, launch4;
     int grid2, grid3, grid4, n_wait, sticky_mask;
     FastChunks fast;
+    bool overlap2;
 };
 StickySizes plan_sticky_step(const StickyInputs& in);
```

Measured after the change: 109,400 (median of 6 runs). 7.4% higher.
